# hpcaitech/CachedEmbedding

Hardware: AMD Instinct MI355X
Metric: embedding lookups/sec (cache op + EmbeddingBag fwd + bwd/SGD), Criteo-1TB table @1% cache (higher is better)
Workload: dtype f32

## Files before the change

cachedembedding_amd/_lib.py:

```python
from __future__ import annotations

import ctypes
import os
from ctypes import POINTER, Structure, c_char_p, c_double, c_float, c_int, c_int32, c_int64, c_size_t, c_uint64, c_void_p
from pathlib import Path

import torch

_PKG = Path(__file__).resolve().parent
LIB_PATH = Path(os.environ["CE_LIBRARY"]) if os.environ.get("CE_LIBRARY") else _PKG / "libce_hip.so"

CE_OK = 0
CE_ERR_INVALID = 1
CE_ERR_HIP = 2
CE_ERR_CAPACITY = 3
CE_ERR_NOMEM = 4
CE_ERR_UNSUPPORTED = 5
CE_ERR_RANGE = 6
CE_EVICT_DATASET = 0
CE_EVICT_LFU = 1
CE_EVICT_LRU = 2
CE_MODE_SUM = 0
CE_MODE_MEAN = 1
CE_ACT_F32 = 0
# ... 106 lines not shown
    "ce_bag_forward_src_keys_act": (c_int, _TABLE + [c_int64] + _KEYS + [c_void_p] + _ACT + _STREAM),
    "ce_bag_backward_dense_act": (c_int, _BAG + _ACT + _KEYS + _STREAM),
    "ce_bag_backward_sgd_act": (c_int, _BAG + _ACT + [c_float] + _KEYS + _STREAM),
    "ce_bag_backward_sgd_src_act": (c_int, _SRC + _ACT + [c_float] + _KEYS + [c_void_p] + _STREAM),
    "ce_bag_backward_dense_src_act": (c_int, _SRC + _ACT + _KEYS + _STREAM),
    "ce_bag_backward_rowwise_adagrad_act": (c_int, _BAG + _ACT + _ADAGRAD_TAIL),
    "ce_bag_backward_rowwise_adagrad_src_act": (c_int, _SRC + _ACT + _ADAGRAD_TAIL),
    "ce_host_fill_uniform_w16": (c_int, [c_void_p, c_int64, c_float, c_float, c_uint64, c_int32, c_int]),
    "ce_bag_forward_w16": (c_int, _W16 + _BAG[1:] + _ACT + _STREAM),
    "ce_bag_forward_src_keys_w16": (c_int, _W16 + [c_int64, c_int32, c_int64] + _KEYS + [c_void_p] + _ACT + _STREAM),
    "ce_bag_backward_w16_workspace": (c_size_t, [c_int64, c_int32]),
    "ce_bag_backward_update_w16": (c_int, _W16 + _BAG[1:] + _ACT + _W16_TAIL),
    "ce_bag_backward_update_src_w16": (c_int, _W16 + _SRC[1:] + _ACT + _W16_TAIL),
    "ce_bag_backward_update_sorted_workspace": (c_size_t, [c_int64, c_int64, c_int32]),
    "ce_bag_backward_update_sorted": (c_int, _W16 + _BAG[1:] + _ACT + _W16_TAIL[1:]),
    "ce_bag_backward_update_compact_workspace": (c_size_t, [c_int64, c_int64, c_int32]),
    "ce_bag_backward_update_compact": (c_int, _W16 + _BAG[1:] + _ACT + _W16_TAIL),
    "ce_bag_backward_update_compact_src": (c_int, _W16 + _SRC[1:] + _ACT + _W16_TAIL),
    "ce_bag_backward_sgd_lrdev": (c_int, _BAG + _ACT + [c_void_p] + _KEYS + _STREAM),
    "ce_bag_backward_sgd_src_lrdev": (c_int, _SRC + _ACT + [c_void_p] + _KEYS + [c_void_p] + _STREAM),
    "ce_bag_backward_update_lrdev": (c_int, _W16 + _BAG[1:] + _ACT + _LRDEV_TAIL),
    "ce_bag_backward_update_src_lrdev": (c_int, _W16 + _SRC[1:] + _ACT + _LRDEV_TAIL),
    "ce_q8_row_bytes": (c_size_t, [c_int32]),
    "ce_host_quantize_q8": (c_int, [c_void_p, c_int32, c_int64, c_int32, c_void_p, c_int]),
    "ce_host_dequantize_q8": (c_int, [c_void_p, c_int64, c_int32, c_void_p, c_int]),
    "ce_bag_forward_q8": (c_int, _BAG + _ACT + _STREAM),
    "ce_bag_forward_src_keys_q8": (c_int, _TABLE + [c_int64] + _KEYS + [c_void_p] + _ACT + _STREAM),
    "ce_q4_row_bytes": (c_size_t, [c_int32]),
    "ce_host_quantize_q4": (c_int, [c_void_p, c_int32, c_int64, c_int32, c_void_p, c_int]),
    "ce_host_dequantize_q4": (c_int, [c_void_p, c_int64, c_int32, c_void_p, c_int]),
    "ce_bag_forward_q4": (c_int, _BAG + _ACT + _STREAM),
    "ce_bag_forward_src_keys_q4": (c_int, _TABLE + [c_int64] + _KEYS + [c_void_p] + _ACT + _STREAM),
    "ce_cache_workspace_bytes": (c_size_t, [c_int64, c_int64, c_int64, c_int32]),
    "ce_cache_create": (c_int, [POINTER(CeCacheConfig), c_void_p, POINTER(c_void_p)]),
    "ce_cache_destroy": (c_int, [c_void_p]),
    "ce_cache_preload": (c_int, [c_void_p, c_void_p, c_void_p, c_int64, c_void_p]),
    "ce_cache_set_freq_bound": (c_int, [c_void_p, c_int64]),
    "ce_cache_prepare_ids": (c_int, [c_void_p, c_void_p, c_int64, c_void_p, c_void_p]),
    "ce_cache_prepare_ids_keys": (c_int, [c_void_p, c_void_p, c_int64, c_int64, c_void_p, c_int32, c_void_p, c_int32,
                                          c_int64, c_int64, c_int32, c_int64, c_void_p, c_void_p]),
    "ce_cache_prepare_ids_begin": (c_int, [c_void_p, c_void_p, c_int64, c_int64, c_void_p, c_int32, c_void_p, c_int32,
                                           c_int64, c_int64, c_int32, c_int64, c_void_p, c_void_p]),
    "ce_cache_prepare_ids_finish": (c_int, [c_void_p, c_void_p]),
    "ce_cache_prepare_ids_padded": (c_int, [c_void_p, c_void_p, c_int64, c_void_p, c_void_p]),
    "ce_cache_prepare_ids_begin_padded": (c_int, [c_void_p, c_void_p, c_int64, c_void_p, c_void_p]),
    "ce_cache_set_deferred_rows": (c_int, [c_void_p, c_int32]),
    "ce_cache_rows_ticket": (c_int64, [c_void_p]),
    "ce_cache_wait_rows": (c_int, [c_void_p, c_int64, c_void_p]),
    "ce_cache_last_stats": (c_int, [c_void_p, POINTER(CeCallStats)]),
    "ce_cache_totals": (c_int, [c_void_p, POINTER(c_int64), POINTER(c_int64), POINTER(c_int64),
                                POINTER(c_int64), POINTER(c_int64)]),
    "ce_cache_history": (c_int64, [c_void_p, c_int64, POINTER(CeCallStats), c_int64]),
    "ce_cache_lookup_slots": (c_int, [c_void_p, c_void_p, c_int64, c_void_p, c_void_p]),
    "ce_cache_flush": (c_int, [c_void_p, c_void_p]),
    "ce_cache_set_protect_depth": (c_int, [c_void_p, c_int32]),
    "ce_cache_set_transport": (c_int, [c_void_p, c_int32]),
    "ce_cache_get_transport": (c_int32, [c_void_p]),
    "ce_cache_set_cache_weight": (c_int, [c_void_p, c_void_p]),
    "ce_cache_graph_replayed": (c_int, [c_void_p, c_int64, c_int64, c_void_p]),
    "ce_cache_set_buffer_rows": (c_int, [c_void_p, c_int64]),
    "ce_cache_set_profiling": (c_int, [c_void_p, c_int32]),
    "ce_cache_phase_count": (c_int32, []),
    "ce_cache_phase_name": (c_char_p, [c_int32]),
    "ce_cache_phase_times": (c_int, [c_void_p, POINTER(c_double), c_int32, POINTER(c_int64), c_int32]),
    "ce_cache_writeback_wait": (c_int, [c_void_p]),
    "ce_cache_swap_stats": (c_int, [c_void_p, POINTER(c_double), POINTER(c_int64)]),
    "ce_cache_failures": (c_int, [c_void_p, POINTER(c_int64), POINTER(c_int32), POINTER(c_int64)]),
    "ce_cache_free_rows": (c_int, [c_void_p, POINTER(c_int64)]),
    "ce_bucketize_workspace": (c_size_t, [c_int64, c_int32]),
    "ce_bucketize_rows": (c_int, [c_void_p, c_int64, c_void_p, c_int32, c_void_p, c_void_p, c_void_p, c_void_p,
                                  c_size_t, c_void_p]),
    "ce_dedupe_bucket_rows": (c_int, [c_void_p, c_int64, c_void_p, c_int64, c_int32, c_void_p, c_void_p,
                                      c_void_p, c_void_p, c_void_p, c_void_p, c_void_p]),
    "ce_dedupe_bucket_rows_padded": (c_int, [c_void_p, c_int64, c_void_p, c_int64, c_int32, c_int64, c_void_p, c_void_p,
                                             c_void_p, c_void_p, c_void_p, c_void_p, c_void_p, c_void_p]),
    "ce_dedupe_bucket_rows_padded_window": (c_int, [c_void_p, c_int64, c_int64, c_void_p, c_int64, c_int32, c_int64,
                                                    c_void_p, c_void_p, c_void_p, c_void_p, c_void_p, c_void_p,
                                                    c_void_p, c_void_p]),
    "ce_exchange_local_index": (c_int, [c_void_p, c_int64, c_int64, c_void_p, c_int64, c_int64, c_int64, c_int64,
                                        c_void_p, c_void_p]),
    "ce_split_classify": (c_int, [c_void_p, c_int32, c_int32, c_int64, c_int64, c_void_p, c_int64, c_void_p, c_void_p,
                                  c_void_p]),
    "ce_split_places": (c_int, [c_void_p, c_void_p, c_int32, c_int32, c_int64, c_int32, c_void_p, c_void_p, c_void_p,
                                c_void_p, c_void_p, c_void_p]),
    "ce_exchange_local_index_split": (c_int, [c_void_p, c_int64, c_int64, c_void_p, c_void_p, c_void_p, c_int64, c_int64,
                                              c_int64, c_int64, c_int64, c_void_p, c_int32, c_int64, c_int64, c_int64,
                                              c_void_p, c_void_p, c_void_p]),
    "ce_bag_forward_max": (c_int, _LOOKUPS + [c_int64, c_void_p, c_void_p] + _STREAM),
    "ce_bag_backward_max": (c_int, [c_void_p, c_int64, c_int32, c_void_p, c_int64, c_int64, c_int64, c_void_p, c_void_p,
                                    c_float, c_void_p]),
    "ce_bag_backward_psw": (c_int, _LOOKUPS + [c_int64, c_void_p, c_void_p] + _STREAM),
    "ce_rows_renorm_workspace": (c_size_t, [c_int64]),
    "ce_rows_renorm": (c_int, [c_void_p, c_int64, c_int32, c_void_p, c_int64, c_float, c_float, c_void_p, c_size_t,
                               c_void_p]),
    "ce_rows_axpy": (c_int, [c_void_p, c_int64, c_int32, c_void_p, c_int64, c_void_p, c_float, c_void_p]),
}


class CeError(RuntimeError):
    def __init__(self, code: int, msg: str):
        super().__init__(f"libce_hip error {code}: {msg}")
        self.code = code


def _load() -> ctypes.CDLL:
    if not LIB_PATH.exists():
# ... 129 lines not shown
```

cachedembedding_amd/cache_mgr.py:

```python
from __future__ import annotations

import ctypes
import math
import weakref
from enum import Enum
from typing import List, Optional

import numpy as np
import torch

from . import _lib
from ._lib import CeCacheConfig, CeCallStats, check, lib, ptr, stream_ptr


class EvictionStrategy(Enum):
    LFU = 1
    DATASET = 2
    LRU = 3


EVICT_CODES = {EvictionStrategy.DATASET: _lib.CE_EVICT_DATASET, EvictionStrategy.LFU: _lib.CE_EVICT_LFU,
               EvictionStrategy.LRU: _lib.CE_EVICT_LRU}


# ... 100 lines not shown
            check(lib.ce_host_fill_uniform_w16(ctypes.c_void_p(self.host_ptr), self.tensor.numel(), lo, hi, seed,
                                               _lib.ACT_DTYPES[self.tensor.dtype], threads or _default_threads()))
            return self
        check(lib.ce_host_fill_uniform(ctypes.c_void_p(self.host_ptr), self.tensor.numel(), lo, hi, seed,
                                       threads or _default_threads()))
        return self


def _default_threads() -> int:
    import os
    return max(1, min(64, (os.cpu_count() or 1)))


class CachedParamMgr(torch.nn.Module):

    def __init__(self, weight, cuda_row_num: int = 0, buffer_size: int = 0, pin_weight: bool = True,
                 evict_strategy: EvictionStrategy = EvictionStrategy.DATASET, async_copy: bool = False,
                 device: Optional[torch.device] = None, strict: bool = True, use_idx_map: Optional[bool] = None):
        super().__init__()
        _lib.require_gpu()
        if cuda_row_num == 0:
            raise NotImplementedError("cuda_row_num == 0 (no cache) is not implemented")
        self._table = weight if isinstance(weight, HostTable) else HostTable.wrap(weight)
        self._weight = self._table.tensor
        self.num_embeddings, self._row_width = self._weight.shape
        self.quant_bits = self._table.quant_bits
        self.table_dtype = _lib.Q4 if self.quant_bits == 4 else self._weight.dtype
        q8 = self.quant_bits != 0
        self.embedding_dim = (2 * (self._row_width - _lib.CE_Q4_HEADER_BYTES) if self.quant_bits == 4
                              else self._row_width - _lib.CE_Q8_HEADER_BYTES) if q8 else self._row_width
        self._lib_dim = self._row_width // 4 if q8 else (
            self.embedding_dim // 2 if self.table_dtype in _lib.W16_DTYPES else self.embedding_dim)
        self.cuda_row_num = int(cuda_row_num)
        self.buffer_size = buffer_size
        self.pin_weight = pin_weight
        self._evict_strategy = evict_strategy
        self._async_copy = async_copy
        self.strict = strict
        self.device = torch.device(device) if device is not None else torch.device("cuda", torch.cuda.current_device())
        N, C, D = self.num_embeddings, self.cuda_row_num, self.embedding_dim
        assert N < 2 ** 31 - 1, "row ids are int32 on the device"
        dev = self.device
        self.cuda_cached_weight = torch.nn.Parameter(
            torch.zeros(C, self._row_width, device=dev, dtype=self._weight.dtype), requires_grad=not q8)
        self._idx_map: Optional[torch.Tensor] = None
        if use_idx_map:
            self._idx_map = torch.arange(N, device=dev, dtype=torch.int32)
        self.register_buffer("cached_idx_map", torch.empty(C, device=dev, dtype=torch.int32), persistent=False)
        self.register_buffer("inverted_cached_idx", torch.empty(N, device=dev, dtype=torch.int32), persistent=False)
        if evict_strategy == EvictionStrategy.LFU:
            self.register_buffer("freq_cnter", torch.empty(C, device=dev, dtype=torch.int64), persistent=False)
        else:
            self.freq_cnter = None
        self._max_ids = 2 ** 31 - 2
        self._deferred_rows = False
        self._handle = None
        self._workspace = None
        self._create_handle()
        self._hist_seen = 0
        self._failures_seen = 0
        self.num_hits_history: List[int] = []
        self.num_miss_history: List[int] = []
        self.num_write_back_history: List[int] = []

    def _create_handle(self):
        N, C = self.num_embeddings, self.cuda_row_num
        ws_bytes = lib.ce_cache_workspace_bytes(N, C, self._max_ids, self._lib_dim)
        self._workspace = torch.empty(ws_bytes + 256, dtype=torch.uint8, device=self.device)
        base = self._workspace.data_ptr()
        aligned = (base + 255) & ~255
        cfg = CeCacheConfig()
        cfg.num_embeddings = N
        cfg.cuda_row_num = C
        cfg.embedding_dim = self._lib_dim
        cfg.evict_strategy = EVICT_CODES[self._evict_strategy]
        tr = getattr(self, "_transport", None)
        cfg.transport = tr if tr is not None else (
            _lib.CE_TRANSPORT_STAGED if self._async_copy else _lib.CE_TRANSPORT_ZEROCOPY)
        reapply_worker = cfg.transport == _lib.CE_TRANSPORT_WORKER
        if reapply_worker:
            cfg.transport = _lib.CE_TRANSPORT_ZEROCOPY
        cfg.protect_depth = 0
        cfg.max_ids_per_call = self._max_ids
        cfg.host_weight = self._table.host_ptr
        cfg.host_weight_dev = self._table.dev_ptr
        cfg.cache_weight = self.cuda_cached_weight.data_ptr()
        cfg.idx_map = ptr(self._idx_map)
        cfg.inverted_cached_idx = self.inverted_cached_idx.data_ptr()
        cfg.cached_idx_map = self.cached_idx_map.data_ptr()
        cfg.freq_cnter = ptr(self.freq_cnter)
        cfg.workspace = aligned
        cfg.workspace_bytes = ws_bytes
        h = ctypes.c_void_p()
        with torch.cuda.device(self.device):
            check(lib.ce_cache_create(ctypes.byref(cfg), stream_ptr(), ctypes.byref(h)))
        self._handle = h
        self._fin = weakref.finalize(self, lib.ce_cache_destroy, h)
        if self.buffer_size and self.buffer_size > 0:
            check(lib.ce_cache_set_buffer_rows(h, int(self.buffer_size)))
        if reapply_worker:
            self.set_transport("worker")

    @property
    def weight(self) -> torch.Tensor:
        if self._handle is not None:
            check(lib.ce_cache_writeback_wait(self._handle))
        return self._weight

    @property
    def idx_map(self) -> torch.Tensor:
        if self._idx_map is None:
            return torch.arange(self.num_embeddings, device=self.device, dtype=torch.int32)
        return self._idx_map

    @property
    def cuda_available_row_num(self) -> int:
        out = ctypes.c_int64()
        check(lib.ce_cache_free_rows(self._handle, ctypes.byref(out)))
        return out.value

    @torch.no_grad()
    def reorder(self, ids_freq_mapping=None, warmup_ratio: float = 0.7):
        N, C = self.num_embeddings, self.cuda_row_num
        freq = None
        order = None
        if ids_freq_mapping is not None:
            freq = torch.as_tensor(ids_freq_mapping).to(device=self.device, dtype=torch.int64).view(-1)
            assert freq.numel() == N
            order = torch.argsort(freq, descending=True, stable=True)
            if self._evict_strategy == EvictionStrategy.DATASET:
                inv = torch.empty(N, device=self.device, dtype=torch.int32)
                inv[order] = torch.arange(N, device=self.device, dtype=torch.int32)
                if self._idx_map is None:
                    self._idx_map = inv
                    self._recreate_with_idx_map()
                else:
                    self._idx_map.copy_(inv)
        n = min(int(math.ceil(C * warmup_ratio)), N)
        if n > 0:
            rows = None
            fvals = None
            if self._evict_strategy in (EvictionStrategy.LFU, EvictionStrategy.LRU) and freq is not None:
                rows = order[:n].to(torch.int32).contiguous()
                if self._evict_strategy == EvictionStrategy.LFU:
                    fvals = freq[order[:n]].contiguous()
            with torch.cuda.device(self.device):
                check(lib.ce_cache_preload(self._handle, ptr(rows), ptr(fvals), n, stream_ptr()))
                if fvals is not None:
                    check(lib.ce_cache_set_freq_bound(self._handle, int(fvals.max().item())))
                torch.cuda.current_stream().synchronize()

    def _recreate_with_idx_map(self):
        assert self.cuda_available_row_num == self.cuda_row_num, "reorder() after rows were cached"
        self._fin.detach()
        lib.ce_cache_destroy(self._handle)
        self._create_handle()
        self._hist_seen = 0
        self._failures_seen = 0

    @torch.no_grad()
    def prepare_ids(self, ids: torch.Tensor, out: Optional[torch.Tensor] = None, padded: bool = False,
                    defer_rows: bool = False) -> torch.Tensor:
        assert ids.is_cuda, "ids must live on the GPU (recsys/dlrm_main.py:250 moves the batch first)"
        shape = ids.shape
        flat = ids if (ids.dim() == 1 and ids.dtype == torch.int64 and ids.is_contiguous()) \
            else ids.reshape(-1).long().contiguous()
        if out is None:
            slots = torch.empty_like(flat)
        else:
            assert out.is_cuda and out.dtype == torch.int64 and out.is_contiguous() and out.numel() == flat.numel()
            slots = out if out.dim() == 1 else out.view(-1)
        fn = lib.ce_cache_prepare_ids_padded if padded else lib.ce_cache_prepare_ids
        if torch.cuda.current_device() == self.device.index:
            check(fn(self._handle, ptr(flat), flat.numel(), ptr(slots), stream_ptr()))
        else:
            with torch.cuda.device(self.device):
                check(fn(self._handle, ptr(flat), flat.numel(), ptr(slots), stream_ptr()))
        if self._deferred_rows and not defer_rows:
            self.wait_rows()
        self._strict_check()
        return slots if slots.shape == shape else slots.view(shape)

    def _strict_check(self) -> None:
        if self.strict and not torch.cuda.is_current_stream_capturing():
            st = CeCallStats()
            rc = lib.ce_cache_last_stats(self._handle, ctypes.byref(st))
            self._pull_history()
            if rc != _lib.CE_OK:
                self._failures_seen += 1
            if rc == _lib.CE_ERR_CAPACITY:
                raise AssertionError(_lib.last_error())
            if rc == _lib.CE_ERR_RANGE:
                raise IndexError(_lib.last_error())
            check(rc)

    @torch.no_grad()
    def prepare_ids_begin(self, ids: torch.Tensor, out: torch.Tensor, keys_out: Optional[torch.Tensor] = None, **layout):
        return self.prepare_ids_keys(ids, out, keys_out, _begin_only=True, **layout)

    @torch.no_grad()
    def prepare_ids_begin_padded(self, ids: torch.Tensor, out: torch.Tensor) -> torch.Tensor:
        assert ids.is_cuda and ids.dtype == torch.int64 and ids.is_contiguous()
        assert out.is_cuda and out.dtype == torch.int64 and out.is_contiguous() and out.numel() == ids.numel()
# ... 232 lines not shown
```

cachedembedding_amd/cached_embedding.py:

```python
from __future__ import annotations

from typing import Callable, Iterator, List, Optional, Tuple, Union

import torch
import torch.nn as nn

from . import _lib
from .cache_mgr import CachedParamMgr, EvictionStrategy, HostTable
from .functional import FusedRowwiseAdagrad, FusedSGD, check_accumulator, check_lr, check_lr_path, embedding_bag


def _refuse_q8_update(module, what: str, lr) -> None:
    if lr is not None and getattr(module, "table_dtype", None) == _lib.Q8:
        raise NotImplementedError(f"{what}(lr) with a q8 (torch.uint8) table: a quantized table is never updated")
    if lr is not None and getattr(module, "table_dtype", None) == _lib.Q4:
        raise NotImplementedError(f"{what}(lr) with a q4 (torch.quint4x2) table: a quantized table is never updated")


def _quant_name(bits: int) -> str:
    return "q4 (torch.quint4x2)" if bits == 4 else "q8 (torch.uint8)"


class CachedEmbeddingBag(nn.Module):
    def __init__(self, num_embeddings: int, embedding_dim: int, padding_idx: Optional[int] = None,
# ... 41 lines not shown
            if padding_idx > 0:
                assert padding_idx < num_embeddings, "Padding_idx must be within num_embeddings"
            elif padding_idx < 0:
                assert padding_idx >= -num_embeddings, "Padding_idx must be within num_embeddings"
                padding_idx = num_embeddings + padding_idx
        self.padding_idx = padding_idx
        self.max_norm = max_norm
        self.norm_type = norm_type
        self.scale_grad_by_freq = scale_grad_by_freq
        self.sparse = sparse
        self.mode = mode
        self.include_last_offset = include_last_offset
        self.evict_strategy = evict_strategy
        self.cache_ratio = cache_ratio
        self.cuda_row_num = int(num_embeddings * cache_ratio) if cuda_row_num is None else int(cuda_row_num)
        self.pool_str = mode
        self.cache_op = True
        self.fused_sgd = FusedSGD(None)
        self.fused_adagrad = FusedRowwiseAdagrad(None)

        if _table is not None:
            table = _table
            assert table.tensor.dtype == (torch.uint8 if q8 else self.table_dtype) and table.quant_bits == bits \
                and table.tensor.shape[0] == num_embeddings
        elif q8:
            w = _weight.detach()
            if w.dtype == torch.uint8:
                width = _lib.q4_row_bytes(embedding_dim) if bits == 4 else _lib.q8_row_bytes(embedding_dim)
                assert tuple(w.shape) == (num_embeddings, width)
                table = HostTable.wrap(w if w.device.type == "cpu" and w.is_contiguous() else w.cpu().contiguous(),
                                       quant_bits=bits)
            else:
                assert tuple(w.shape) == (num_embeddings, embedding_dim)
                if w.dtype not in _lib.ACT_DTYPES:
                    w = w.float()
                table = HostTable.allocate(num_embeddings, embedding_dim, dtype=self.table_dtype).quantize_from(
                    w.cpu().contiguous())
        elif _weight is None:
            table = HostTable.allocate(num_embeddings, embedding_dim, dtype=self.table_dtype)
            table.fill_uniform_(-1.0 / num_embeddings, 1.0 / num_embeddings, init_seed)
            if padding_idx is not None:
                table.tensor[padding_idx].zero_()
        else:
            w = _weight.detach()
            assert tuple(w.shape) == (num_embeddings, embedding_dim)
            if w.device.type != "cpu" or w.dtype != self.table_dtype or not w.is_contiguous():
                w = w.to("cpu", self.table_dtype).contiguous()
            table = HostTable.wrap(w)
        self.cache_weight_mgr = CachedParamMgr(table, self.cuda_row_num, buffer_size, pin_weight,
                                               evict_strategy=evict_strategy, device=device, strict=strict,
                                               use_idx_map=True if _idx_map is not None else None)
        if _idx_map is not None:
            self.cache_weight_mgr._idx_map.copy_(_idx_map)
        self.cache_weight_mgr.reorder(ids_freq_mapping, warmup_ratio)
        if q8:
            self.eval()
        if w16:
            self.set_weight_rounding(self.weight_rounding, self.weight_rounding_seed)

    @property
    def weight(self) -> torch.Tensor:
        return self.cache_weight_mgr.weight

    def named_parameters(self, prefix: str = "", recurse: bool = True, remove_duplicate: bool = True
                         ) -> Iterator[Tuple[str, nn.Parameter]]:
        yield (prefix + ("." if prefix else "") + "weight", self.cache_weight_mgr.cuda_cached_weight)

    def parameters(self, recurse: bool = True) -> Iterator[nn.Parameter]:
        yield self.cache_weight_mgr.cuda_cached_weight

    def set_cache_op(self, cache_op: bool = True):
        self.cache_op = cache_op

    def set_cache_mgr_async_copy(self, flag: bool):
        self.cache_weight_mgr.set_async_copy(flag)

    def set_fused_sgd(self, lr: Union[float, torch.Tensor, None], deterministic: bool = False,
                      accumulator: str = "cache"):
        _refuse_q8_update(self, "set_fused_sgd", lr)
        if isinstance(lr, torch.Tensor):
            check_lr_path(check_lr(lr), bool(deterministic), self.mode)
        if lr is not None or accumulator != "step":
            check_accumulator("sgd", self.table_dtype, accumulator, bool(deterministic), self.weight_rounding)
        if lr is not None and self.fused_adagrad.lr is not None:
            raise ValueError("fused row-wise Adagrad is set: set_fused_rowwise_adagrad(None) before set_fused_sgd(lr)")
        if lr is not None and deterministic and self.table_dtype != torch.float32:
            raise NotImplementedError("FusedSGD(deterministic=True) with a 16-bit table")
        self.fused_sgd.lr = lr
        self.fused_sgd.deterministic = deterministic
        self.fused_sgd.accumulator = accumulator

    def set_fused_rowwise_adagrad(self, lr: Union[float, torch.Tensor, None], eps: float = 1e-8,
                                  deterministic: bool = False, accumulator: str = "cache"):
        _refuse_q8_update(self, "set_fused_rowwise_adagrad", lr)
        if isinstance(lr, torch.Tensor):
            check_lr_path(check_lr(lr), bool(deterministic), self.mode)
        if lr is not None or accumulator != "step":
            check_accumulator("rowwise_adagrad", self.table_dtype, accumulator, bool(deterministic),
                              self.weight_rounding)
        if lr is not None and self.fused_sgd.lr is not None:
            raise ValueError("fused SGD is set: set_fused_sgd(None) before set_fused_rowwise_adagrad(lr)")
        mgr = self.cache_weight_mgr
        if lr is not None and getattr(mgr, "momentum1", None) is None:
            mgr.momentum1 = torch.zeros(mgr.num_embeddings, device=mgr.device, dtype=torch.float32)
        self.fused_adagrad.lr = lr
        self.fused_adagrad.eps = float(eps)
# ... 112 lines not shown
```

cachedembedding_amd/csrc/ce_bag.hip:

```cpp
#include <algorithm>

#include "ce_common.h"

namespace ce {

struct BagParams {
  const float* weight;
  float* dst;
  const void* grad_out;
  const int64_t* indices;
  const void* offsets;
  const float* psw;
  int64_t nnz;
  int32_t num_bags;
  int32_t rowlen;
  int32_t g_log2;
  int32_t off64;
  int32_t include_last;
  int32_t mode;
  int32_t hookF;
  int32_t hookB;
  float alpha;
  int32_t pad0;
  uint32_t num_rows;
// ... 373 lines not shown
__device__ __forceinline__ void tile_sort_1024(KT (&key)[4], KT* lds, int tid) {
  for (int k = 2; k <= kBwdTile; k <<= 1) {
    for (int j = k >> 1; j > 0; j >>= 1) {
      if (j >= 256) {
#pragma unroll
        for (int r = 0; r < 4; ++r) lds[tid * 4 + r] = key[r];
        __syncthreads();
#pragma unroll
        for (int r = 0; r < 4; ++r) {
          const int i = tid * 4 + r;
          const KT other = lds[i ^ j];
          const bool lower = (i & j) == 0, up = (i & k) == 0;
          const KT lo = key[r] < other ? key[r] : other, hi = key[r] < other ? other : key[r];
          key[r] = (lower == up) ? lo : hi;
        }
        __syncthreads();
      } else if (j >= 4) {
#pragma unroll
        for (int r = 0; r < 4; ++r) {
          const int i = tid * 4 + r;
          const KT other = shfl_xor_key<KT>(key[r], j >> 2);
          const bool lower = (i & j) == 0, up = (i & k) == 0;
          const KT lo = key[r] < other ? key[r] : other, hi = key[r] < other ? other : key[r];
          key[r] = (lower == up) ? lo : hi;
        }
      } else {
#pragma unroll
        for (int r = 0; r < 4; ++r) {
          if (r & j) continue;
          const bool up = ((tid * 4 + r) & k) == 0;
          const KT a = key[r], b = key[r | j];
          if ((a > b) == up) {
            key[r] = b;
            key[r | j] = a;
          }
        }
      }
    }
  }
#pragma unroll
  for (int r = 0; r < 4; ++r) lds[tid * 4 + r] = key[r];
  __syncthreads();
}

constexpr int kSegLen = 16384;
constexpr int kSegKeys = 16;
#ifndef CE_SEG_BUCKETS
#define CE_SEG_BUCKETS 8192
#endif
constexpr int kSegBuckets = CE_SEG_BUCKETS;
constexpr int kExclRun = 32;
constexpr unsigned kExclFlag = 0x80000000u;

template <bool SRC, bool EXCL, bool ROWS>
__global__ __launch_bounds__(1024) void k_bag_presort_seg(const int64_t* __restrict__ indices, int64_t nnz_per_batch,
                                                         int32_t segs_per_batch, int64_t n_segs, uint32_t num_rows,
                                                         unsigned long long* __restrict__ keys_out, BagParams lay,
                                                         int64_t off_stride, const int64_t* __restrict__ ids,
                                                         int64_t* __restrict__ ids_minmax, int64_t* slots_io,
                                                         const int32_t* __restrict__ inverted,
                                                         const int* __restrict__ status) {
  __shared__ unsigned long long lk[kSegLen];
  static_assert(sizeof(unsigned long long) * kSegLen <= 160 * 1024 - 1024, "gfx950: 160 KB of LDS per CU");
  int* const cnt = (int*)lk;
  __shared__ int wsum[16];
  __shared__ long long mm_s[2][16];
  const int tid = threadIdx.x, lane = tid & 63, wv = tid >> 6;
  for (int64_t seg = blockIdx.x; seg < n_segs; seg += gridDim.x) {
    const int64_t batch = seg / segs_per_batch;
    const int sib = (int)(seg - batch * segs_per_batch);
    const int64_t in_base = batch * nnz_per_batch + (int64_t)sib * kSegLen;
    const int64_t base = seg * kSegLen;
    const int n_here = (int)min((int64_t)kSegLen, nnz_per_batch - (int64_t)sib * kSegLen);
    BagParams q = lay;
    if (SRC && lay.offsets) q.offsets = (const char*)lay.offsets + batch * off_stride * (lay.off64 ? 8 : 4);
    for (int i = tid; i <= kSegBuckets; i += 1024) cnt[i] = 0;
    __syncthreads();
    unsigned long long key[kSegKeys];
    int place[kSegKeys], bkt[kSegKeys];
    int32_t slot_r[ROWS ? kSegKeys : 1];
    if (ROWS) {
      const bool failed = *status != CE_OK;
      int32_t row_r[kSegKeys];
#pragma unroll
      for (int r = 0; r < kSegKeys; ++r) {
        const int e = r * 1024 + tid;
        row_r[r] = e < n_here ? (int32_t)slots_io[in_base + e] : -1;
      }
#pragma unroll
      for (int r = 0; r < kSegKeys; ++r) slot_r[r] = (row_r[r] >= 0 && !failed) ? inverted[row_r[r]] : -1;
#pragma unroll
      for (int r = 0; r < kSegKeys; ++r) {
        const int e = r * 1024 + tid;
        if (e < n_here) slots_io[in_base + e] = (int64_t)slot_r[r];
      }
    }
#pragma unroll
    for (int r = 0; r < kSegKeys; ++r) {
      const int e = r * 1024 + tid;
      key[r] = ~0ull;
      bkt[r] = kSegBuckets;
      if (e < n_here) {
        const int64_t row = ROWS ? (int64_t)slot_r[ROWS ? r : 0] : indices[in_base + e];
        const bool valid = (uint64_t)row < (uint64_t)num_rows;
        if (valid || SRC) {
          unsigned low = (unsigned)e;
          if (SRC)
            low = (unsigned)out_row(q, lay.offsets ? find_bag(q, sib * kSegLen + e) : sib * kSegLen + e);
          key[r] = ((unsigned long long)(valid ? (uint32_t)row : 0xffffffffu) << 32) | low;
          if (valid) bkt[r] = (int)(row & (kSegBuckets - 1));
        }
      }
      const int b0 = __builtin_amdgcn_readfirstlane(bkt[r]);
      if (__all(bkt[r] == b0)) {
        int first = 0;
        if (lane == 0) first = atomicAdd(&cnt[b0], 64);
        place[r] = __shfl(first, 0) + lane;
      } else {
        place[r] = atomicAdd(&cnt[bkt[r]], 1);
      }
    }
    __syncthreads();
    constexpr int kPer = kSegBuckets / 1024;
    int c4[kPer], sum = 0;
#pragma unroll
    for (int q = 0; q < kPer; ++q) { c4[q] = cnt[tid * kPer + q]; sum += c4[q]; }
    int inc = sum;
#pragma unroll
    for (int d = 1; d < 64; d <<= 1) {
      const int o = __shfl_up(inc, d);
      if (lane >= d) inc += o;
    }
    if (lane == 63) wsum[wv] = inc;
    __syncthreads();
    int pre = inc - sum;
    for (int k = 0; k < wv; ++k) pre += wsum[k];
    int total = 0;
    for (int k = 0; k < 16; ++k) total += wsum[k];
#pragma unroll
    for (int q = 0; q < kPer; ++q) { cnt[tid * kPer + q] = pre; pre += c4[q]; }
    if (tid == 0) cnt[kSegBuckets] = total;
    __syncthreads();
    if (!EXCL) {
// ... 937 lines not shown
  return launch_fwd_keys(weight, kTableQ8, num_rows, dim, true, nnz, src_keys, out, act_dtype, (hipStream_t)stream);
}

#define CE_REQUIRE_Q4_DIM(dim)                                                         \
  CE_REQUIRE(ce_q4_row_bytes(dim) != 0, CE_ERR_UNSUPPORTED,                            \
             "a q4 table needs dim %% 32 == 0 and 32 <= dim <= 1024 (got %d)", (int)(dim))
#define CE_REQUIRE_Q4_ALIGNED(weight, out, act)                                        \
  CE_REQUIRE(al16(weight) && act_aligned(out, act), CE_ERR_INVALID,                    \
             "a q4 table must be 16-byte aligned and its output on the vector boundary")

extern "C" int ce_bag_forward_q4(const void* weight, int64_t num_rows, int32_t dim, const int64_t* indices, int64_t nnz,
                                 const void* offsets, int32_t offsets_are_i64, int64_t num_bags,
                                 int32_t include_last_offset, const float* per_sample_weights, int32_t mode,
                                 int64_t hook_features, void* out, int32_t act_dtype, ce_stream_t stream) {
  CE_REQUIRE_ACT(act_dtype);
  CE_REQUIRE_Q4_DIM(dim);
  if (num_bags == 0) return CE_OK;
  CE_REQUIRE(weight && out && (indices || nnz == 0), CE_ERR_INVALID, "null pointer");
  CE_REQUIRE(offsets || num_bags == nnz, CE_ERR_INVALID,
             "offsets == NULL states one id per bag (offsets = arange): num_bags must equal nnz");
  CE_REQUIRE_Q4_ALIGNED(weight, out, act_dtype);
  BagParams p{};
  RowGeom r;
  int rc = fill_params(p, r, dim, true, indices, nnz, offsets, offsets_are_i64, num_bags, include_last_offset,
                       per_sample_weights, mode, hook_features);
  if (rc) return rc;
  return launch_fwd(p, r, weight, kTableQ4, num_rows, out, act_dtype, (hipStream_t)stream);
}

extern "C" int ce_bag_forward_src_keys_q4(const void* weight, int64_t num_rows, int32_t dim, int64_t nnz,
                                          const uint64_t* src_keys, void* out, int32_t act_dtype, ce_stream_t stream) {
  CE_REQUIRE_ACT(act_dtype);
  CE_REQUIRE_Q4_DIM(dim);
  if (nnz == 0) return CE_OK;
  CE_REQUIRE(weight && src_keys && out, CE_ERR_INVALID, "null pointer");
  CE_REQUIRE_ROWS(num_rows);
  CE_REQUIRE_Q4_ALIGNED(weight, out, act_dtype);
  return launch_fwd_keys(weight, kTableQ4, num_rows, dim, true, nnz, src_keys, out, act_dtype, (hipStream_t)stream);
}

extern "C" int64_t ce_bag_presort_len(int64_t nnz) { return nnz <= 0 ? 0 : padded_keys(nnz); }

static int window_layout(BagParams& lay, const BagLayout& L, const int64_t* indices, int64_t nnz_per_batch) {
  CE_REQUIRE(L.num_bags > 0 && L.offsets_batch_stride >= 0, CE_ERR_INVALID, "bad offsets");
  CE_REQUIRE(L.offsets || L.num_bags == nnz_per_batch, CE_ERR_INVALID,
             "offsets may only be NULL for the one-id-per-bag layout (num_bags == nnz_per_batch)");
  RowGeom unused;
  return fill_params(lay, unused, 4, true, indices, nnz_per_batch, L.offsets, L.offsets_are_i64, L.num_bags,
                     L.include_last_offset, nullptr, CE_MODE_SUM, L.hook_features);
}

static int launch_presort(const int64_t* indices, int64_t* slots_io, const int32_t* inverted, const int* status,
                          int64_t nnz_per_batch, int64_t n_batches, int64_t num_rows, const BagLayout* L,
                          const int64_t* ids, int64_t* ids_minmax, uint64_t* keys_out, hipStream_t s) {
  if (nnz_per_batch == 0 || n_batches == 0) return CE_OK;
  CE_REQUIRE((slots_io ? inverted && status : indices != nullptr) && keys_out && nnz_per_batch > 0 && n_batches > 0,
             CE_ERR_INVALID, "bad arguments");
  CE_REQUIRE(nnz_per_batch < (int64_t)INT32_MAX - kSegLen, CE_ERR_INVALID, "batch too large");
  CE_REQUIRE_ROWS(num_rows);
  const int64_t spb = cdiv(nnz_per_batch, kSegLen);
  const int64_t nseg = spb * n_batches;
  CE_REQUIRE(spb < (int64_t)INT32_MAX && nseg < (int64_t)INT32_MAX, CE_ERR_INVALID, "too many segments");
  BagParams lay{};
  if (L) {
    int rc = window_layout(lay, *L, indices, nnz_per_batch);
    if (rc) return rc;
  }
  const dim3 grid((unsigned)std::min<int64_t>(nseg, kMaxBlocks)), block(1024);
  const int64_t off_stride = L ? L->offsets_batch_stride : 0;
  auto launch = [&](auto src, auto excl, auto rows) {
    hipLaunchKernelGGL((k_bag_presort_seg<decltype(src)::value, decltype(excl)::value, decltype(rows)::value>), grid, block,
                       0, s, indices, nnz_per_batch, (int32_t)spb, nseg, (uint32_t)num_rows,
                       (unsigned long long*)keys_out, lay, off_stride, ids, ids_minmax, slots_io, inverted, status);
  };
  const std::true_type yes{};
  const std::false_type no{};
  if (slots_io && L) launch(yes, no, yes);
  else if (slots_io) launch(no, no, yes);
  else if (L && ids_minmax) launch(yes, yes, no);
  else if (L) launch(yes, no, no);
  else launch(no, no, no);
  CE_LAUNCH_CHECK();
  return CE_OK;
}

namespace ce {
int presort_window_from_rows(int64_t* slots_io, int64_t nnz_per_batch, int64_t n_batches, int64_t num_rows,
                             const int32_t* inverted, const int* status, int32_t src_keys, const BagLayout& lay,
                             uint64_t* keys_out, hipStream_t stream) {
  return launch_presort(nullptr, slots_io, inverted, status, nnz_per_batch, n_batches, num_rows, src_keys ? &lay : nullptr,
                        nullptr, nullptr, keys_out, stream);
}
}

extern "C" int ce_bag_presort_window(const int64_t* indices, int64_t nnz_per_batch, int64_t n_batches,
                                     int64_t num_rows, uint64_t* keys_out, ce_stream_t stream) {
  return launch_presort(indices, nullptr, nullptr, nullptr, nnz_per_batch, n_batches, num_rows, nullptr, nullptr, nullptr,
                        keys_out, (hipStream_t)stream);
}

static int presort_window_src_impl(const int64_t* indices, int64_t nnz_per_batch, int64_t n_batches, int64_t num_rows,
                                   const BagLayout& L, const int64_t* ids, uint64_t* keys_out, int64_t* seg_id_ranges,
                                   ce_stream_t stream) {
  if (nnz_per_batch == 0 || n_batches == 0) return CE_OK;
  BagParams lay{};
  int rc = window_layout(lay, L, indices, nnz_per_batch);
  if (rc) return rc;
  return launch_presort(indices, nullptr, nullptr, nullptr, nnz_per_batch, n_batches, num_rows, &L, ids, seg_id_ranges,
                        keys_out, (hipStream_t)stream);
}

extern "C" int ce_bag_presort_window_src(const int64_t* indices, int64_t nnz_per_batch, int64_t n_batches,
                                         int64_t num_rows, const void* offsets, int32_t offsets_are_i64,
                                         int64_t offsets_batch_stride, int64_t num_bags, int32_t include_last_offset,
                                         int64_t hook_features, uint64_t* keys_out, ce_stream_t stream) {
  return presort_window_src_impl(indices, nnz_per_batch, n_batches, num_rows,
                                 {offsets, offsets_are_i64, offsets_batch_stride, num_bags, include_last_offset, hook_features},
                                 nullptr, keys_out, nullptr, stream);
}

extern "C" int ce_bag_presort_window_src_excl(const int64_t* indices, int64_t nnz_per_batch, int64_t n_batches,
                                              int64_t num_rows, const void* offsets, int32_t offsets_are_i64,
                                              int64_t offsets_batch_stride, int64_t num_bags,
                                              int32_t include_last_offset, int64_t hook_features, const int64_t* ids,
                                              uint64_t* keys_out, int64_t* seg_id_ranges, ce_stream_t stream) {
  CE_REQUIRE(seg_id_ranges, CE_ERR_INVALID, "null seg_id_ranges");
  return presort_window_src_impl(indices, nnz_per_batch, n_batches, num_rows,
                                 {offsets, offsets_are_i64, offsets_batch_stride, num_bags, include_last_offset, hook_features},
                                 ids, keys_out, seg_id_ranges, stream);
}

extern "C" int ce_bag_presort(const int64_t* indices, int64_t nnz, int64_t num_rows, uint64_t* keys_out,
                              ce_stream_t stream) {
  return ce_bag_presort_window(indices, nnz, 1, num_rows, keys_out, stream);
}

extern "C" int ce_rows_axpy(float* weight, int64_t num_rows, int32_t dim, const int64_t* index, int64_t n,
                            const float* src_rows, float alpha, ce_stream_t stream) {
  if (n == 0) return CE_OK;
  CE_REQUIRE(weight && index && src_rows, CE_ERR_INVALID, "null pointer");
  CE_REQUIRE(dim > 0 && n > 0 && n < (int64_t)INT32_MAX, CE_ERR_INVALID, "bad sizes");
  CE_REQUIRE_ROWS(num_rows);
  RowGeom r;
  int rc = row_geometry(dim, al16(weight) && al16(src_rows), r);
// ... 36 lines not shown
```

cachedembedding_amd/csrc/ce_cache.hip:

```cpp
#include <sched.h>
#include <stdlib.h>
#include <string.h>
#include <sys/prctl.h>

#include <algorithm>
#include <atomic>
#include <chrono>
#include <condition_variable>
#include <functional>
#include <mutex>
#include <thread>
#include <vector>

#include "ce_common.h"

#include "ce_cache_index.h"
#include "ce_cache_select.h"
#include "ce_cache_rows.h"
#include "ce_cache_fused.h"
#include "ce_cache_worker.h"


struct KeysTail {
  int64_t n_batches, nnz_per_batch;
// ... 10 lines not shown
  ce::Ctl* ctl = nullptr;
  uint32_t* bitmap = nullptr;
  int32_t *blk_unique = nullptr, *blk_miss = nullptr, *coarse = nullptr, *miss_list = nullptr, *slot_epoch = nullptr,
          *victims = nullptr, *blk_free = nullptr, *free_list = nullptr;
  int32_t* miss_list_b[2] = {};
  int32_t* free_list_b[2] = {};
  ce::ChainWords* chain = nullptr;
  unsigned long long *lb_emit = nullptr, *lb_remap = nullptr;
  unsigned lb_tag = 0;
  ce::FrontWords* front = nullptr;
  int32_t *fine_cnt = nullptr, *coarse_cnt = nullptr;
  long long front_calls = 0;
  bool front_cleanup_pending = false;
  unsigned long long* keys = nullptr;
  uint32_t* hist = nullptr;
  ce_call_stats_t* ring = nullptr;
  ce_call_stats_t* ring_dev = nullptr;
  hipEvent_t ev = nullptr;
  float* stage = nullptr;
  int32_t* stage_idx = nullptr;
  long long seq = 0;
  long long drained = 0;
  std::vector<ce_call_stats_t> history;
  int64_t cpu_to_cuda_numel = 0, cuda_to_cpu_numel = 0, cache_miss = 0, total_cache = 0;
  int vec = 0;
  int rowlen = 0, g_log2 = 0, slot_bits = 0, word_bits = 0;
  int host_threads = 1;
  float* stage_dev = nullptr;
  float* stage_host = nullptr;
  int32_t* list_host = nullptr;
  ce::Ctl* ctl_host = nullptr;
  int64_t stage_rows = 0;
  int64_t list_rows = 0;
  int64_t buffer_rows = 0;
  ce::RowPool* pool = nullptr;
  ce::SwapEngine* wb = nullptr;
  unsigned long long* evt_keys[2] = {};
  int32_t* evt_pos[2] = {};
  uint32_t evt_mask = 0;
  float* stage2 = nullptr;
  int32_t* stage_idx2 = nullptr;
  float* in_stage = nullptr;
  long long hist_base = 1;
  ce::PhaseProf* prof = nullptr;
  uint64_t freq_bound = 0;
  uint64_t graph_freq_limit = ~0ull;
  bool freq_bound_known = true;
  long long n_failed = 0;
  int last_fail_status = CE_OK;
  long long last_fail_seq = 0;
  bool free_zero = false;
  long long free_reset_seq = 0;
  bool deferred_rows = false;
  struct Pending {
    bool active = false;
    int64_t n = 0;
    int64_t* slots_out = nullptr;
    hipStream_t s = nullptr;
    bool worker = false, capturing = false, has_tail = false;
    bool chained = false;
    long long call = 0;
    int parity = 0;
    long long in_job = 0, seq_arg = 0;
    int cap_groups = 1, swap_threads = 256;
    bool sel_pending = false;
    bool sel_steady = false;
    long long sel_out_job = 0;
    int sel_wbuf = 0;
    int pslot = 0, pmark = 0;
    const void* prof = nullptr;
    KeysTail tail{};
  } pend;
};

using namespace ce;

template <typename VT_> struct RowTag { typedef VT_ VT; };
template <typename F> static inline void for_rows(const ce_cache* h, F&& f) {
  if (h->vec) f(RowTag<f32x4>{}); else f(RowTag<float>{});
}

static PhaseProf* live_prof(const ce_cache* h) {
  return (h->prof && (const void*)h->prof == h->pend.prof) ? h->prof : nullptr;
}
static void phase_mark(ce_cache* h) {
  ce_cache::Pending& x = h->pend;
  if (PhaseProf* const prof = live_prof(h)) (void)hipEventRecord(prof->ev[x.pslot][x.pmark++], x.s);
}

static int ensure_writeback(ce_cache* h);

static void drain(ce_cache* h) {
  while (h->drained < h->seq) {
    const long long s = h->drained + 1;
    const ce_call_stats_t& r = h->ring[s % kRing];
    if (r.seq != s) break;
    if (h->history.empty()) h->hist_base = s;
    h->history.push_back(r);
    if (h->history.size() > (size_t)2 * kHistoryKeep) {
      h->history.erase(h->history.begin(), h->history.end() - kHistoryKeep);
      h->hist_base = h->history.front().seq;
    }
    if (r.status != CE_OK) {
      h->n_failed += 1;
      h->last_fail_status = r.status;
      h->last_fail_seq = s;
      h->free_zero = false;
      h->free_reset_seq = h->seq;
    } else if (r.kind == CE_CALL_PREPARE && s > h->free_reset_seq) {
      h->free_zero = r.n_free_after == 0;
    }
    if (r.status == CE_OK && r.kind != CE_CALL_PRELOAD) {
      h->cpu_to_cuda_numel += r.n_miss * h->cfg.embedding_dim;
      h->cuda_to_cpu_numel += r.n_evict * h->cfg.embedding_dim;
      h->cache_miss += r.miss_lookups;
      h->total_cache += r.n_ids;
      if (h->wb && h->wb->chained && r.kind == CE_CALL_PREPARE) {
        std::lock_guard<std::mutex> g(h->wb->m);
        h->wb->in_rows += r.n_miss;
      }
    }
    h->drained = s;
  }
}

static hipEvent_t last_rows_event(ce_cache* h) {
  if (!h->wb || !h->wb->chained || h->wb->chain_calls == 0) return nullptr;
  return h->wb->ev_rows[h->wb->chain_calls % SwapEngine::kRowsRing];
}
static int join_rows(ce_cache* h, hipStream_t s) {
  if (hipEvent_t ev = last_rows_event(h)) CE_HIP_CHECK(hipStreamWaitEvent(s, ev, 0));
  return CE_OK;
}
// ... 314 lines not shown
    static const int out_threads = [] { const char* e = getenv("CE_WB_THREADS"); return e ? atoi(e) : dflt; }();
    static const int in_threads = [] { const char* e = getenv("CE_GATHER_THREADS"); return e ? atoi(e) : dflt; }();
    w->out_pool = new RowPool(std::max(1, std::min(out_threads, 64)));
    w->in_pool = new RowPool(std::max(1, std::min(in_threads, 64)));
    w->rowlen = h->rowlen;
    w->g_log2 = h->g_log2;
    w->vec = h->vec;
    w->out_thread = std::thread([w] { w->run_out(); });
    if (!w->chained) w->in_thread = std::thread([w] { w->run_in(); });
  } while (0);
  if (rc) {
    delete w;
    set_error("swap worker setup failed (pinned buffers / streams / events)");
    return rc;
  }
  h->wb = w;
  return CE_OK;
}

extern "C" int ce_cache_set_freq_bound(ce_cache_t* h, int64_t bound) {
  CE_REQUIRE(h && bound >= 0, CE_ERR_INVALID, "bad bound");
  if (h->cfg.evict_strategy == CE_EVICT_LRU) return CE_OK;
  h->freq_bound = std::max<uint64_t>(h->freq_bound, (uint64_t)bound);
  h->freq_bound_known = true;
  return CE_OK;
}

extern "C" int ce_cache_preload(ce_cache_t* h, const int32_t* rows, const int64_t* freq_vals, int64_t n,
                                ce_stream_t stream) {
  CE_REQUIRE(h, CE_ERR_INVALID, "null handle");
  CE_REQUIRE(n >= 0 && n <= h->cfg.cuda_row_num, CE_ERR_INVALID, "preload count out of range");
  CE_REQUIRE(!h->pend.active, CE_ERR_INVALID, "a cache op begun with ce_cache_prepare_ids_begin has not been finished");
  if (n == 0) return CE_OK;
  if (freq_vals && h->cfg.evict_strategy != CE_EVICT_LRU) h->freq_bound_known = false;
  int rc = before_call(h);
  if (rc) return rc;
  if (h->wb) {
    rc = h->wb->wait_out(h->wb->out_issued);
    if (rc) return rc;
  }
  hipStream_t s = (hipStream_t)stream;
  const ce_cache_config_t& c = h->cfg;
  rc = join_rows(h, s);
  if (rc) return rc;
  h->seq += 1;
  const int64_t groups_per_block = 256 >> h->g_log2;
  for_rows(h, [&](auto r) {
    using VT = typename decltype(r)::VT;
    hipLaunchKernelGGL((k_admit<VT>), dim3(grid_for(n, (int)groups_per_block * kSwapRows)), dim3(256), 0, s, rows,
                       (const int32_t*)nullptr, (const long long*)nullptr, (long long)n, (const VT*)c.host_weight_dev,
                       (VT*)c.cache_weight, h->rowlen, h->g_log2, (const Ctl*)nullptr, 0ll);
  });
  hipLaunchKernelGGL(k_admit_maps, dim3(grid_for(n, 256)), dim3(256), 0, s, rows, (const int32_t*)nullptr,
                     (const long long*)nullptr, (long long)n, c.cached_idx_map, c.inverted_cached_idx,
                     c.freq_cnter, freq_vals, h->slot_epoch, kEpochNever, (Ctl*)nullptr,
                     (ce_call_stats_t*)nullptr, 0ll, (const unsigned long long*)nullptr, 0ll);
  hipLaunchKernelGGL(k_preload_end, dim3(1), dim3(1), 0, s, (long long)n, h->ctl, h->ring_dev + (h->seq % kRing),
                     h->seq);
  CE_LAUNCH_CHECK();
  CE_HIP_CHECK(hipEventRecord(h->ev, s));
  return CE_OK;
}

static int worker_selftest(ce_cache* h, hipStream_t s) {
  SwapEngine* w = h->wb;
  if (w->tested && w->tested_stream == s) return CE_OK;
  CE_HIP_CHECK(hipStreamSynchronize(s));
  unsigned long long* word = w->sig + 2;
  __atomic_store_n(word, 0ull, __ATOMIC_RELEASE);
  CE_HIP_CHECK(hipStreamWaitValue64(s, word, 1, hipStreamWaitValueGte, ~0ull));
  std::this_thread::sleep_for(std::chrono::milliseconds(2));
  hipError_t e = hipMemcpyAsync(w->rows_host[0], w->stage_dev[0], 64, hipMemcpyDeviceToHost, w->out_stream);
  if (e == hipSuccess) e = hipMemcpyAsync(w->rows_host[1], w->stage_dev[1], 64, hipMemcpyDeviceToHost, w->out_stream2);
  if (e == hipSuccess) e = hipMemcpyAsync(w->in_stage_dev, w->rows_host[0], 64, hipMemcpyHostToDevice, w->in_stream);
  bool done = e == hipSuccess;
  if (done) {
    for (hipStream_t st : {w->out_stream, w->out_stream2, w->in_stream})
      if (stream_wait_polite(st, 0.25) != hipSuccess) done = false;
  }
  __atomic_store_n(word, 1ull, __ATOMIC_RELEASE);
  CE_HIP_CHECK(hipStreamSynchronize(s));
  if (e != hipSuccess) {
    set_error("worker transport self-test: %s", hipGetErrorString(e));
    return CE_ERR_HIP;
  }
  if (!done) {
    set_error("worker transport self-test failed: copies on the library's copy streams do not run while the cache-op "
              "stream is parked in hipStreamWaitValue64 (they share a hardware queue with it: GPU_MAX_HW_QUEUES = %s)",
              getenv("GPU_MAX_HW_QUEUES") ? getenv("GPU_MAX_HW_QUEUES") : "unset");
    return CE_ERR_UNSUPPORTED;
  }
  w->tested = true;
  w->tested_stream = s;
  return CE_OK;
}

struct FrontTail {
  const int32_t* miss_tmp;
  const FrontWords* fw;
  uint32_t* bitmap;
  int32_t *fine, *coarse;
};
static FrontTail take_front_tail(ce_cache* h) {
  if (!h->front_cleanup_pending) return FrontTail{nullptr, nullptr, nullptr, nullptr, nullptr};
  h->front_cleanup_pending = false;
  return FrontTail{h->victims, h->front + (h->front_calls & 1), h->bitmap, h->fine_cnt, h->coarse_cnt};
}
// ... 15 lines not shown
    if (capturing) {
      bound = h->freq_bound + kGraphFreqHeadroom;
      h->graph_freq_limit = bound;
    } else {
      h->freq_bound = bound;
    }
    const int bits = 64 - __builtin_clzll(bound | 1ull) + h->slot_bits;
    top_pass = h->freq_bound_known ? std::min(kLevels - 1, std::max(0, (bits + kDigitBits - 1) / kDigitBits - 1))
                                   : kLevels - 1;
  }
  return top_pass;
}

static int launch_keys_hist(ce_cache* h) {
  const ce_cache::Pending& x = h->pend;
  const ce_cache_config_t& c = h->cfg;
  const int64_t N = c.num_embeddings, C = c.cuda_row_num;
  const int top_pass = select_top_pass(h, x.n, x.capturing);
  const FrontTail ft = take_front_tail(h);
  const auto keys_kernel = c.evict_strategy == CE_EVICT_LRU   ? k_keys<CE_EVICT_LRU>
                           : c.evict_strategy == CE_EVICT_LFU ? k_keys<CE_EVICT_LFU>
                                                              : k_keys<CE_EVICT_DATASET>;
  hipLaunchKernelGGL(keys_kernel, dim3(std::min(grid_for(C, 256 * 4), 512)), dim3(256), 0, x.s, c.cached_idx_map, c.freq_cnter,
                     h->slot_epoch, C, N, x.seq_arg, c.protect_depth, h->slot_bits, top_pass, h->keys, h->hist, h->ctl,
                     ft.miss_tmp, ft.fw, ft.bitmap, ft.fine, ft.coarse, (int)h->L.n_chunks);
  const int hgrid = (int)std::min<int64_t>(kNumCU, std::max<int64_t>(1, cdiv(C, 1024 * 4)));
  for (int pass = top_pass - 1; pass >= 0; --pass)
    hipLaunchKernelGGL(k_hist, dim3(hgrid), dim3(1024), 0, x.s, h->keys, C, pass, top_pass, h->hist, h->ctl);
  return top_pass;
}


static int64_t staged_chunk(const ce_cache* h, int64_t rows) {
  return (h->buffer_rows > 0 && h->buffer_rows < rows) ? h->buffer_rows : rows;
}
static size_t rowbytes(const ce_cache* h) { return (size_t)h->cfg.embedding_dim * sizeof(float); }

static int staged_swap(ce_cache* h, hipStream_t s) {
  const ce_cache_config_t& c = h->cfg;
  const int D = c.embedding_dim;
  if (!h->ctl_host) CE_HIP_CHECK(hipHostMalloc((void**)&h->ctl_host, sizeof(Ctl), hipHostMallocDefault));
  CE_HIP_CHECK(hipMemcpyAsync(h->ctl_host, h->ctl, sizeof(Ctl), hipMemcpyDeviceToHost, s));
  CE_HIP_CHECK(hipStreamSynchronize(s));
  const Ctl ctl = *h->ctl_host;
  if (ctl.status != CE_OK) return CE_OK;
  const int64_t k = ctl.k_evict, m = ctl.n_miss;
  const int64_t big = std::max<int64_t>(std::max(k, m), 1);
  int rc = ensure_staging(h, staged_chunk(h, big), big);
  if (rc) return rc;
  const int gpb = 256 >> h->g_log2;
  if (k > 0) {
    int32_t* evicted_rows_dev = h->free_list;
    hipLaunchKernelGGL(k_evict_maps, dim3(grid_for(k, 256)), dim3(256), 0, s, h->victims, c.cached_idx_map,
                       c.inverted_cached_idx, evicted_rows_dev, h->ctl);
    CE_HIP_CHECK(hipMemcpyAsync(h->list_host, evicted_rows_dev, (size_t)k * 4, hipMemcpyDeviceToHost, s));
    const int64_t chunk = staged_chunk(h, k);
    for (int64_t off = 0; off < k; off += chunk) {
      const int64_t cnt = std::min(chunk, k - off);
      for_rows(h, [&](auto r) {
        using VT = typename decltype(r)::VT;
        hipLaunchKernelGGL((k_pack_rows<VT>), dim3(grid_for(cnt, gpb)), dim3(256), 0, s, (const int32_t*)h->victims + off,
                           (long long)cnt, (const VT*)c.cache_weight, (VT*)h->stage_dev, h->rowlen, h->g_log2);
      });
      CE_HIP_CHECK(hipMemcpyAsync(h->stage_host, h->stage_dev, (size_t)cnt * rowbytes(h), hipMemcpyDeviceToHost, s));
      CE_HIP_CHECK(hipStreamSynchronize(s));
      float* table = c.host_weight;
      const float* st = h->stage_host;
      const int32_t* rows = h->list_host + off;
      const size_t rb = rowbytes(h);
      host_pool(h)->parallel(cnt, [=](int64_t lo, int64_t hi) {
        for (int64_t i = lo; i < hi; ++i) memcpy(table + (size_t)rows[i] * D, st + (size_t)i * D, rb);
      });
    }
  }
  return CE_OK;
}

static int admit_staged(ce_cache* h) {
  const ce_cache_config_t& c = h->cfg;
  hipStream_t s = h->pend.s;
  const Ctl ctl = *h->ctl_host;
  const int64_t m = (ctl.status == CE_OK) ? ctl.n_miss : 0;
  if (m <= 0) return CE_OK;
  const int D = c.embedding_dim, gpb = 256 >> h->g_log2;
  const size_t rb = rowbytes(h);
  CE_HIP_CHECK(hipMemcpyAsync(h->list_host, h->miss_list, (size_t)m * 4, hipMemcpyDeviceToHost, s));
  CE_HIP_CHECK(hipStreamSynchronize(s));
  const float* table = c.host_weight;
  float* st = h->stage_host;
  const int64_t chunk = staged_chunk(h, m);
  for (int64_t off = 0; off < m; off += chunk) {
    const int64_t cnt = std::min(chunk, m - off);
    if (off > 0) CE_HIP_CHECK(hipStreamSynchronize(s));
    const int32_t* rows = h->list_host + off;
    host_pool(h)->parallel(cnt, [=](int64_t lo, int64_t hi) {
      for (int64_t i = lo; i < hi; ++i) memcpy(st + (size_t)i * D, table + (size_t)rows[i] * D, rb);
    });
    CE_HIP_CHECK(hipMemcpyAsync(h->stage_dev, h->stage_host, (size_t)cnt * rb, hipMemcpyHostToDevice, s));
    for_rows(h, [&](auto r) {
      using VT = typename decltype(r)::VT;
      hipLaunchKernelGGL((k_unpack_rows<VT>), dim3(grid_for(cnt, gpb)), dim3(256), 0, s, (const int32_t*)h->free_list + off,
                         (long long)cnt, (const VT*)h->stage_dev, (VT*)c.cache_weight, h->rowlen, h->g_log2);
    });
  }
  return CE_OK;
}

static int select_and_stage(ce_cache* h) {
  const ce_cache::Pending& x = h->pend;
  const ce_cache_config_t& c = h->cfg;
  const Layout& L = h->L;
  const int64_t C = c.cuda_row_num;
  hipStream_t s = x.s;
  const bool worker = x.worker, steady = x.sel_steady;
  const int wbuf = x.sel_wbuf, n_vblocks = (int)cdiv(C, 4096), gpb = 256 >> h->g_log2;
  int32_t* const free_list = h->free_list_b[x.chained ? x.parity : 0];
  const int top_pass = launch_keys_hist(h);
  hipLaunchKernelGGL(k_victims, dim3((unsigned)n_vblocks), dim3(256), 0, s, h->keys, C, h->victims, L.list_cap, h->ctl,
                     (const uint32_t*)h->hist, top_pass, h->ring_dev, x.seq_arg, steady ? h->blk_free : (int32_t*)nullptr);
  phase_mark(h);
  if (c.transport == CE_TRANSPORT_ZEROCOPY || worker) {
    float* const stage_cur = (worker && wbuf) ? h->stage2 : h->stage;
    int32_t* const stage_idx_cur = (worker && wbuf) ? h->stage_idx2 : h->stage_idx;
    const long long scap = (long long)L.stage_rows;
    const int sgrid = (int)std::min<int64_t>(512, std::max<int64_t>(1, cdiv(L.stage_rows, gpb)));
    WbMail* const mail = worker ? h->wb->mail_dev + wbuf : nullptr;
    const dim3 sg(sgrid + (steady ? n_vblocks : 0));
    const EvTable evt = (worker && h->wb->chained) ? EvTable{h->evt_keys[wbuf], h->evt_pos[wbuf], h->evt_mask}
                                                     : EvTable{nullptr, nullptr, 0u};
    for_rows(h, [&](auto r) {
      using VT = typename decltype(r)::VT;
      hipLaunchKernelGGL((k_evict_stage<VT>), sg, dim3(256), 0, s, h->victims, c.cached_idx_map, c.inverted_cached_idx,
                         (const VT*)c.cache_weight, (VT*)stage_cur, stage_idx_cur, scap, h->rowlen, h->g_log2, h->ctl, mail,
                         x.sel_out_job, sgrid, (const unsigned long long*)h->keys, C, (const int32_t*)h->blk_free, free_list,
                         evt, L.list_cap > L.stage_rows ? (VT*)c.host_weight_dev : (VT*)nullptr);
    });
    if (worker) {
      CE_HIP_CHECK(hipEventRecord(h->wb->out_ev[wbuf], s));
      h->wb->push_out();
    }
  } else {
    const int rc = staged_swap(h, s);
    if (rc) return rc;
  }
  phase_mark(h);
  if (steady) {
  } else if (C <= 16384) {
    hipLaunchKernelGGL(k_free_single, dim3(1), dim3(1024), 0, s, c.cached_idx_map, C, free_list, h->ctl);
  } else {
    hipLaunchKernelGGL(k_free_count, dim3((unsigned)L.n_slot_blocks), dim3(256), 0, s, c.cached_idx_map, C,
                       h->blk_free, h->ctl);
    hipLaunchKernelGGL(k_free_emit, dim3((unsigned)L.n_slot_blocks), dim3(256), 0, s, c.cached_idx_map, C,
                       h->blk_free, free_list, h->ctl);
  }
  phase_mark(h);
  return CE_OK;
}

struct MarkCfg {
  bool merge;
  int u, threads, blocks, hot_words;
};
static MarkCfg mark_cfg(const ce_cache* h, int64_t n) {
  const bool ranked = h->cfg.idx_map != nullptr;
  MarkCfg m;
  m.merge = !ranked;
  m.threads = ranked ? 512 : 256;
  m.hot_words = (int)std::min<int64_t>(h->L.bitmap_words, ranked ? 8192 : 2048);
  m.u = n >= 65536 ? 4 : 1;
  m.blocks = std::min(grid_for(n, m.threads * m.u), 256);
  return m;
}

constexpr int64_t kScanMaxIds = (1 << 23) - 1;

static void launch_front_kernels(ce_cache* h, const int64_t* ids, int64_t n, int64_t* slots_out, hipStream_t s,
                                 int allow_pad, bool steady, long long seq_arg, int32_t* miss_list, WbMail* mail_in,
                                 long long in_job, int32_t* miss_host, long long* n_admit_out, bool single_pass_ok) {
  const ce_cache_config_t& c = h->cfg;
  const Layout& L = h->L;
  const int64_t N = c.num_embeddings, C = c.cuda_row_num;
  if (h->front_cleanup_pending) {
    hipLaunchKernelGGL(k_front_cleanup, dim3(64), dim3(256), 0, s, (const int32_t*)h->victims,
                       (const FrontWords*)(h->front + (h->front_calls & 1)), h->bitmap, h->fine_cnt, h->coarse_cnt,
                       (int)L.n_chunks);
    h->front_cleanup_pending = false;
  }
  if (single_pass_ok && !mail_in && !miss_host && n < (int64_t)INT32_MAX && L.n_chunks <= kRankMaxChunks) {
    const long long fc = ++h->front_calls;
    FrontWords* const fw = h->front + (fc & 1);
    FrontWords* const fw_next = h->front + ((fc + 1) & 1);
    if (n > 0) {
      const int U = n >= 65536 ? 2 : 1;
      const int threads = (int)std::min<int64_t>(1024, std::max<int64_t>(64, cdiv(cdiv(n, U), 64) * 64));
      const dim3 tg((unsigned)cdiv(n, (int64_t)threads * U)), tb(threads);
#define CE_TOUCH(U_)                                                                                                \
  hipLaunchKernelGGL((k_touch<U_>), tg, tb, 0, s, ids, n, c.idx_map, c.inverted_cached_idx, N, h->bitmap, h->fine_cnt, \
                     h->coarse_cnt, h->slot_epoch, seq_arg, fw, h->victims, (unsigned)L.list_cap, slots_out, allow_pad)
      if (U == 2) CE_TOUCH(2); else CE_TOUCH(1);
#undef CE_TOUCH
    }
    const int rgrid = (int)std::min<int64_t>(kNumCU, std::max<int64_t>(1, cdiv(std::max(n, C), 4096)));
    hipLaunchKernelGGL(k_miss_rank, dim3(rgrid), dim3(256), (size_t)L.n_chunks * 4, s, (const int32_t*)h->victims, fw, fw_next,
                       (const uint32_t*)h->bitmap, (const int32_t*)h->fine_cnt, (const int32_t*)h->coarse_cnt,
                       (int)L.n_chunks, (unsigned)L.list_cap, miss_list, (const int32_t*)h->slot_epoch, C, h->hist, seq_arg, h->ctl, n, h->ring_dev,
                       (long long)L.stage_rows, steady ? 1 : 0, n_admit_out);
    h->front_cleanup_pending = true;
    return;
  }
  hipLaunchKernelGGL(k_begin, dim3(16), dim3(256), 0, s, h->ctl, h->coarse,
                     (int)(((L.n_chunks >> kCoarseShift) + 1) * 2 * kCoarsePad), h->hist, seq_arg);
  if (n > 0) {
    const MarkCfg mc = mark_cfg(h, n);
    const dim3 mg(mc.blocks), mb(mc.threads);
#define CE_MARK(M, U_)                                                                                             \
  hipLaunchKernelGGL((k_mark<M, U_>), mg, mb, mc.hot_words * 4, s, ids, n, c.idx_map, c.inverted_cached_idx, N,    \
                     h->word_bits, mc.hot_words, h->bitmap, h->ctl, slots_out, allow_pad)
    if (mc.merge) { if (mc.u == 4) CE_MARK(true, 4); else CE_MARK(true, 1); }
    else { if (mc.u == 4) CE_MARK(false, 4); else CE_MARK(false, 1); }
#undef CE_MARK
  }
  hipLaunchKernelGGL(k_count, dim3((unsigned)L.n_chunks), dim3(256), 0, s, (const uint4*)h->bitmap,
                     c.inverted_cached_idx, N, h->blk_unique, h->blk_miss, h->coarse);
  hipLaunchKernelGGL(k_emit, dim3((unsigned)cdiv(L.n_chunks, kEmitSub)), dim3(256), 0, s, (uint4*)h->bitmap, c.inverted_cached_idx, N,
                     h->blk_miss, h->coarse, (int)L.n_chunks, miss_list, h->slot_epoch, seq_arg, h->ctl, C, n, h->ring_dev,
                     mail_in, in_job, (long long)L.stage_rows, miss_host, steady ? 1 : 0, n_admit_out);
}

static int prepare_ids_second_half(ce_cache* h);
static int chained_second_half(ce_cache* h);
static int launch_slots_keys(ce_cache* h);

static ce_cache::Pending& record_call(ce_cache* h, int64_t n, int64_t* slots_out, hipStream_t s, const KeysTail* tail,
                                      bool worker, bool capturing, int split, long long out_job, long long in_job,
                                      long long chain_call) {
  const ce_cache_config_t& c = h->cfg;
  ce_cache::Pending x;
  x.n = n;
  x.slots_out = slots_out;
  x.s = s;
  x.worker = worker;
  x.capturing = capturing;
  x.has_tail = tail != nullptr;
  if (tail) x.tail = *tail;
  x.chained = chain_call > 0;
  x.call = chain_call;
  x.parity = (int)(chain_call & 1);
  x.in_job = in_job;
  x.seq_arg = capturing ? 0ll : (long long)h->seq;
  const int swap_blocks = c.protect_depth > 0 ? 32 : 512;
  x.swap_threads = 256;
  x.cap_groups = (int)std::min<int64_t>(swap_blocks, std::max<int64_t>(1, cdiv(h->L.list_cap, (x.swap_threads >> h->g_log2) * kSwapRows)));
// ... 28 lines not shown
  {
    const int blocks = n <= 600000 ? 32 : 20;
    const long long prev = out_job - 1;
    const int pb = (int)(prev & 1);
    bool landed;
    {
      std::lock_guard<std::mutex> g(w->m);
      landed = w->out_done >= prev;
      w->in_jobs += 1;
      if (!landed) w->in_probed += 1;
    }
    const bool has_prev = prev >= w->probe_floor && !landed;
    const unsigned long long* ek = has_prev ? h->evt_keys[pb] : nullptr;
    const long long* n_ptr = &h->chain->n_admit[parity];
    for_rows(h, [&](auto r) {
      using VT = typename decltype(r)::VT;
      hipLaunchKernelGGL((k_admit_probe<VT>), dim3(blocks), dim3(1024), 0, w->in_stream, h->miss_list_b[parity], n_ptr,
                         (const VT*)h->cfg.host_weight_dev, (VT*)h->in_stage, h->rowlen, h->g_log2, ek,
                         (const int32_t*)h->evt_pos[pb], h->evt_mask, (uint32_t)prev, (const VT*)(pb ? h->stage2 : h->stage));
    });
  }
  phase_mark(h);
  if (split) {
    x.active = true;
    CE_LAUNCH_CHECK();
    return CE_OK;
  }
  return chained_second_half(h);
}

static int chained_second_half(ce_cache* h) {
  ce_cache::Pending& x = h->pend;
  x.active = false;
  x.sel_pending = false;
  SwapEngine* const w = h->wb;
  const ce_cache_config_t& c = h->cfg;
  const Layout& L = h->L;
  hipStream_t s = x.s;
  const int parity = x.parity, wbuf = x.sel_wbuf, pslot = x.pslot;
  const long long call = x.call, out_job = x.sel_out_job;
  PhaseProf* const prof = live_prof(h);
  if (prof) {
    (void)hipEventRecord(prof->resume[pslot], s);
    prof->resumed[pslot] = true;
  }
  if (call > 1) CE_HIP_CHECK(hipStreamWaitEvent(s, w->ev_rows[(call - 1) % SwapEngine::kRowsRing], 0));
  hipEvent_t sel_done = w->out_ev[wbuf];
  if (x.sel_steady && x.n <= kScanMaxIds) {
    const int64_t C = c.cuda_row_num;
    const int top_pass = launch_keys_hist(h);
    phase_mark(h);
    StageArgs a;
    a.cached_idx_map = c.cached_idx_map;
    a.inverted = c.inverted_cached_idx;
    a.freq = c.freq_cnter;
    a.slot_epoch = h->slot_epoch;
    a.C = C;
    a.seq_arg = x.seq_arg;
    a.top_pass = top_pass;
    a.keys = h->keys;
    a.hist = h->hist;
    a.ctl = h->ctl;
    a.lb = h->lb_remap;
    h->lb_tag = (h->lb_tag + 1) & 0xffffu;
    a.tag = h->lb_tag;
    a.free_list = h->free_list_b[parity];
    a.miss_list = h->miss_list_b[parity];
    a.ring = h->ring_dev;
    a.n_unpack_out = &h->chain->n_unpack[parity];
    a.cache = c.cache_weight;
    a.stage = wbuf ? h->stage2 : h->stage;
    a.stage_rows_idx = wbuf ? h->stage_idx2 : h->stage_idx;
    a.scap = (long long)L.stage_rows;
    a.rowlen = h->rowlen;
    a.g_log2 = h->g_log2;
    a.vec = h->vec;
    a.mail = w->mail_dev + wbuf;
    a.job = out_job;
    a.evt = EvTable{h->evt_keys[wbuf], h->evt_pos[wbuf], h->evt_mask};
    a.host_overflow = L.list_cap > L.stage_rows ? (void*)c.host_weight_dev : nullptr;
    hipLaunchKernelGGL(k_rank_victims, dim3((unsigned)cdiv(C, kRemapSlots)), dim3(256), 0, s, a);
    {
      const int gpb = 256 >> h->g_log2;
      const int sgrid = (int)std::min<int64_t>(x.n <= 600000 ? 256 : 512,
                                               std::max<int64_t>(1, cdiv(L.stage_rows, gpb * kStageRowsInFlight)));
      hipLaunchKernelGGL(k_stage_maps, dim3(sgrid), dim3(256), 0, s, a);
    }
    CE_HIP_CHECK(hipEventRecord(w->out_ev[wbuf], s));
    w->push_out();
    for (int j = 0; j < 2; ++j) phase_mark(h);
  } else {
    int rc0 = select_and_stage(h);
    if (rc0) return rc0;
    hipLaunchKernelGGL(k_admit_maps, dim3(grid_for(L.list_cap, 256)), dim3(256), 0, s, h->miss_list_b[parity],
                       h->free_list_b[parity], (const long long*)&h->ctl->n_miss, 0ll, c.cached_idx_map,
                       c.inverted_cached_idx, c.freq_cnter, (const int64_t*)nullptr, h->slot_epoch, 0, h->ctl,
                       h->ring_dev, x.seq_arg, (const unsigned long long*)nullptr, 0ll, &h->chain->n_unpack[parity]);
    CE_HIP_CHECK(hipEventRecord(w->ev_miss[parity], s));
    sel_done = w->ev_miss[parity];
  }
  CE_HIP_CHECK(hipStreamWaitEvent(w->in_stream, sel_done, 0));
  {
    const int gpb = 256 >> h->g_log2;
    const int ugrid = (int)std::min<int64_t>(x.n <= 600000 ? 128 : 512, std::max<int64_t>(1, cdiv(L.stage_rows, gpb)));
    const long long prev = out_job - 1;
    const int pb = (int)(prev & 1);
    const unsigned long long* ek = prev >= w->probe_floor ? h->evt_keys[pb] : nullptr;
    const bool tail_possible = L.list_cap > L.stage_rows;
    for_rows(h, [&](auto r) {
      using VT = typename decltype(r)::VT;
      hipLaunchKernelGGL((k_unpack_chained<VT>), dim3(ugrid), dim3(256), 0, w->in_stream, h->free_list_b[parity],
                         (const long long*)&h->chain->n_unpack[parity], (long long)L.stage_rows, (const VT*)h->in_stage,
                         (VT*)c.cache_weight, h->rowlen, h->g_log2, (const int32_t*)h->miss_list_b[parity],
                         tail_possible ? (const VT*)c.host_weight_dev : (const VT*)nullptr, ek,
                         (const int32_t*)h->evt_pos[pb], h->evt_mask, (uint32_t)prev, (const VT*)(pb ? h->stage2 : h->stage));
    });
  }
  if (prof) (void)hipEventRecord(prof->adm1[pslot], w->in_stream);
  hipEvent_t rows = w->ev_rows[call % SwapEngine::kRowsRing];
  CE_HIP_CHECK(hipEventRecord(rows, w->in_stream));
  phase_mark(h);
  int rc = launch_slots_keys(h);
  if (rc) return rc;
  if (prof) prof->pending[pslot] = true;
  CE_LAUNCH_CHECK();
  if (!h->deferred_rows) CE_HIP_CHECK(hipStreamWaitEvent(s, rows, 0));
  CE_HIP_CHECK(hipEventRecord(h->ev, s));
  return CE_OK;
}

static int prepare_ids_impl(ce_cache_t* h, const int64_t* ids, int64_t n, int64_t* slots_out, ce_stream_t stream,
                            int allow_pad, const KeysTail* tail = nullptr, int split = 0) {
  CE_REQUIRE(h, CE_ERR_INVALID, "null handle");
  CE_REQUIRE(!h->pend.active, CE_ERR_INVALID, "a cache op begun with ce_cache_prepare_ids_begin has not been finished");
  CE_REQUIRE(n >= 0 && n <= std::max<int64_t>(h->cfg.max_ids_per_call, 0), CE_ERR_INVALID,
             "n=%lld exceeds max_ids_per_call=%lld", (long long)n, (long long)h->cfg.max_ids_per_call);
  CE_REQUIRE(n == 0 || (ids && slots_out), CE_ERR_INVALID, "null ids/slots");
  hipStream_t s = (hipStream_t)stream;
  hipStreamCaptureStatus cap_st = hipStreamCaptureStatusNone;
  if (s != nullptr) CE_HIP_CHECK(hipStreamIsCapturing(s, &cap_st));
  const bool capturing = cap_st == hipStreamCaptureStatusActive;
  if (capturing) {
    CE_REQUIRE(h->cfg.transport == CE_TRANSPORT_ZEROCOPY, CE_ERR_UNSUPPORTED,
               "only the zero-copy transport can be captured in a hipGraph (the others hand rows to host threads)");
    CE_REQUIRE(!h->prof, CE_ERR_UNSUPPORTED, "switch the phase timers off before capturing a cache op");
    CE_REQUIRE(!split, CE_ERR_UNSUPPORTED, "a cache op in two halves cannot be captured in a hipGraph");
  }
  int rc = capturing ? CE_OK : before_call(h);
  if (rc) return rc;
  bool worker = h->cfg.transport == CE_TRANSPORT_WORKER;
  if (worker) {
    rc = ensure_writeback(h);
    if (rc) return rc;
    if (h->wb->chained) {
      rc = h->wb->check();
      if (rc) return rc;
      h->seq += 1;
      return chained_first_half(h, ids, n, slots_out, s, allow_pad, tail, split);
    }
  }
  if (!capturing) h->seq += 1;

  long long out_job = 0, in_job = 0;
  if (worker) {
    rc = worker_selftest(h, s);
    if (rc == CE_ERR_UNSUPPORTED) {
      fprintf(stderr, "[libce_hip] %s -- falling back to the zero-copy transport\n", ce_last_error());
      rc = h->wb->wait_out(h->wb->out_issued);
      if (rc) return rc;
      h->cfg.transport = CE_TRANSPORT_ZEROCOPY;
      worker = false;
    } else if (rc) {
      return rc;
    }
  }
  if (worker) {
    {
      int prio = 0, prio_lo = 0, prio_hi = 0;
      (void)hipDeviceGetStreamPriorityRange(&prio_lo, &prio_hi);
      if (s != nullptr && prio_hi != prio_lo && hipStreamGetPriority(s, &prio) == hipSuccess)
        CE_REQUIRE(prio != prio_hi, CE_ERR_UNSUPPORTED,
                   "the worker transport's host-gather admission cannot run its cache op on a highest-priority stream "
                   "(its copy streams use that priority to stay out of the parked stream's hardware queue)");
    }
    out_job = h->wb->out_issued + 1;
    in_job = h->wb->in_issued + 1;
    rc = h->wb->wait_out(out_job - 2);
    if (rc == CE_OK) rc = h->wb->wait_in(in_job - 2);
    if (rc) return rc;
  }
  ce_cache::Pending& x = record_call(h, n, slots_out, s, tail, worker, capturing, split, out_job, in_job, 0ll);
  if (PhaseProf* const prof = live_prof(h)) prof->collect(x.pslot);
  phase_mark(h);
  launch_front_kernels(h, ids, n, slots_out, s, allow_pad, x.sel_steady, x.seq_arg, h->miss_list,
                       worker ? h->wb->mail_dev + 2 : (WbMail*)nullptr, in_job,
                       worker ? h->wb->miss_host_dev : (int32_t*)nullptr, (long long*)nullptr, !capturing);
  if (worker) {
    CE_HIP_CHECK(hipEventRecord(h->wb->in_ev[in_job & 1], s));
    h->wb->push_in(out_job - 1);
  }
  phase_mark(h);
  if (!x.sel_pending) {
    rc = select_and_stage(h);
    if (rc) return rc;
  }
  if (split) {
    x.active = true;
    CE_LAUNCH_CHECK();
    return CE_OK;
  }
  return prepare_ids_second_half(h);
}

static int launch_slots_keys(ce_cache* h) {
  const ce_cache::Pending& x = h->pend;
  const ce_cache_config_t& c = h->cfg;
  const int64_t C = c.cuda_row_num, n = x.n;
  int64_t* const slots_out = x.slots_out;
  hipStream_t s = x.s;
  const ce_stream_t stream = (ce_stream_t)s;
  const int lfu = c.evict_strategy == CE_EVICT_LFU;
  const KeysTail* const tail = x.has_tail ? &x.tail : nullptr;
  int rc = CE_OK;
  if (n > 0 && lfu) {
    hipLaunchKernelGGL(k_slots_lfu, dim3(std::min(grid_for(n, 8192), kMaxBlocks)), dim3(1024), 0, s, slots_out, n,
                       c.inverted_cached_idx, c.freq_cnter, (const Ctl*)h->ctl);
    if (tail) {
      rc = tail->src_keys
               ? ce_bag_presort_window_src(slots_out, tail->nnz_per_batch, tail->n_batches, C, tail->lay.offsets,
                                           tail->lay.offsets_are_i64, tail->lay.offsets_batch_stride, tail->lay.num_bags,
                                           tail->lay.include_last_offset, tail->lay.hook_features, tail->keys_out, stream)
               : ce_bag_presort_window(slots_out, tail->nnz_per_batch, tail->n_batches, C, tail->keys_out, stream);
      if (rc) return rc;
    }
  } else if (n > 0 && tail) {
    rc = presort_window_from_rows(slots_out, tail->nnz_per_batch, tail->n_batches, C, c.inverted_cached_idx,
                                  &h->ctl->status, tail->src_keys, tail->lay, tail->keys_out, s);
    if (rc) return rc;
  } else if (n > 0) {
    hipLaunchKernelGGL(k_slots, dim3(grid_for(n, 256 * 4)), dim3(256), 0, s, slots_out, n, c.inverted_cached_idx,
                       (const Ctl*)h->ctl);
  }
  phase_mark(h);
  return CE_OK;
}


static int admit_parked(ce_cache* h) {
  const ce_cache::Pending& x = h->pend;
  const ce_cache_config_t& c = h->cfg;
  const Layout& L = h->L;
  const long long scap = (long long)L.stage_rows;
  CE_HIP_CHECK(hipStreamWaitValue64(x.s, h->wb->sig, (uint64_t)x.in_job, hipStreamWaitValueGte, ~0ull));
  const int ugrid = (int)std::min<int64_t>(1024, std::max<int64_t>(1, cdiv(L.stage_rows, 256 >> h->g_log2)));
  for_rows(h, [&](auto r) {
    using VT = typename decltype(r)::VT;
    hipLaunchKernelGGL((k_unpack_admitted<VT>), dim3(ugrid), dim3(256), 0, x.s, h->free_list,
                       (const long long*)&h->ctl->n_miss, scap, (const VT*)h->in_stage, (VT*)c.cache_weight, h->rowlen,
                       h->g_log2, h->ctl, (const unsigned long long*)(h->wb->sig_dev + 1), x.in_job,
                       (const int32_t*)h->miss_list,
                       L.list_cap > L.stage_rows ? (const VT*)c.host_weight_dev : (const VT*)nullptr);
  });
  return CE_OK;
}

static int admit_zero_copy(ce_cache* h) {
  const ce_cache::Pending& x = h->pend;
  const ce_cache_config_t& c = h->cfg;
  const long long scap = (long long)h->L.stage_rows;
  const int cap_groups = x.cap_groups;
  const int wb_groups = c.protect_depth > 0 ? std::max(1, cap_groups / 2) : cap_groups;
  auto swap = [&](auto r, auto rows) {
    using VT = typename decltype(r)::VT;
    hipLaunchKernelGGL((k_swap<VT, decltype(rows)::value>), dim3(wb_groups + cap_groups), dim3(x.swap_threads), 0, x.s,
                       h->stage_idx, (const VT*)h->stage, scap, wb_groups, h->miss_list, h->free_list,
                       (const long long*)&h->ctl->n_miss, (VT*)c.host_weight_dev, (VT*)c.cache_weight, h->rowlen,
                       h->g_log2, (const Ctl*)h->ctl);
  };
  if (h->vec && x.n <= 131072) swap(RowTag<f32x4>{}, std::integral_constant<int, 4>{});
  else for_rows(h, [&](auto r) { swap(r, std::integral_constant<int, 16>{}); });
  return CE_OK;
}

static int prepare_ids_second_half(ce_cache* h) {
  ce_cache::Pending& x = h->pend;
  if (x.chained) return chained_second_half(h);
  x.active = false;
  PhaseProf* const prof = live_prof(h);
  int rc = CE_OK;
  if (x.sel_pending) {
    x.sel_pending = false;
    if (prof) {
      (void)hipEventRecord(prof->resume[x.pslot], x.s);
      prof->resumed[x.pslot] = true;
    }
    rc = select_and_stage(h);
    if (rc) return rc;
  }
  const ce_cache_config_t& c = h->cfg;
  hipStream_t s = x.s;
  rc = x.worker ? admit_parked(h) : c.transport == CE_TRANSPORT_ZEROCOPY ? admit_zero_copy(h) : admit_staged(h);
  if (rc) return rc;
  hipLaunchKernelGGL(k_admit_maps, dim3(grid_for(h->L.list_cap, 256)), dim3(256), 0, s, h->miss_list, h->free_list,
                     (const long long*)&h->ctl->n_miss, 0ll, c.cached_idx_map, c.inverted_cached_idx,
                     c.freq_cnter, (const int64_t*)nullptr, h->slot_epoch, 0, h->ctl, h->ring_dev,
                     x.seq_arg, x.worker ? (const unsigned long long*)(h->wb->sig_dev + 1) : nullptr, x.in_job);
  phase_mark(h);
  rc = launch_slots_keys(h);
  if (rc) return rc;
  if (prof) prof->pending[x.pslot] = true;
  CE_LAUNCH_CHECK();
  if (!x.capturing) CE_HIP_CHECK(hipEventRecord(h->ev, s));
  return CE_OK;
}

extern "C" int ce_cache_prepare_ids(ce_cache_t* h, const int64_t* ids, int64_t n, int64_t* slots_out,
                                    ce_stream_t stream) {
  return prepare_ids_impl(h, ids, n, slots_out, stream, 0);
}

extern "C" int ce_cache_prepare_ids_keys(ce_cache_t* h, const int64_t* ids, int64_t n_batches, int64_t nnz_per_batch,
                                         int64_t* slots_out, int32_t src_keys, const void* offsets,
                                         int32_t offsets_are_i64, int64_t offsets_batch_stride, int64_t num_bags,
                                         int32_t include_last_offset, int64_t hook_features, uint64_t* keys_out,
                                         ce_stream_t stream) {
  CE_REQUIRE(n_batches > 0 && nnz_per_batch > 0 && keys_out, CE_ERR_INVALID, "bad window shape / null keys_out");
  KeysTail t{n_batches, nnz_per_batch, src_keys,
             {offsets, offsets_are_i64, offsets_batch_stride, num_bags, include_last_offset, hook_features}, keys_out};
  return prepare_ids_impl(h, ids, n_batches * nnz_per_batch, slots_out, stream, 0, &t);
}

extern "C" int ce_cache_prepare_ids_begin(ce_cache_t* h, const int64_t* ids, int64_t n_batches, int64_t nnz_per_batch,
                                          int64_t* slots_out, int32_t src_keys, const void* offsets,
                                          int32_t offsets_are_i64, int64_t offsets_batch_stride, int64_t num_bags,
                                          int32_t include_last_offset, int64_t hook_features, uint64_t* keys_out,
                                          ce_stream_t stream) {
  CE_REQUIRE(n_batches > 0 && nnz_per_batch > 0, CE_ERR_INVALID, "bad window shape");
  if (!keys_out) return prepare_ids_impl(h, ids, n_batches * nnz_per_batch, slots_out, stream, 0, nullptr, 1);
  KeysTail t{n_batches, nnz_per_batch, src_keys,
             {offsets, offsets_are_i64, offsets_batch_stride, num_bags, include_last_offset, hook_features}, keys_out};
  return prepare_ids_impl(h, ids, n_batches * nnz_per_batch, slots_out, stream, 0, &t, 1);
}

extern "C" int ce_cache_prepare_ids_finish(ce_cache_t* h, ce_stream_t stream) {
  CE_REQUIRE(h, CE_ERR_INVALID, "null handle");
  CE_REQUIRE(h->pend.active, CE_ERR_INVALID, "no cache op has been begun");
  CE_REQUIRE((hipStream_t)stream == h->pend.s, CE_ERR_INVALID, "finish the cache op on the stream it was begun on");
  return prepare_ids_second_half(h);
}

extern "C" int ce_cache_prepare_ids_padded(ce_cache_t* h, const int64_t* ids, int64_t n, int64_t* slots_out,
                                           ce_stream_t stream) {
  return prepare_ids_impl(h, ids, n, slots_out, stream, 1);
}

extern "C" int ce_cache_prepare_ids_begin_padded(ce_cache_t* h, const int64_t* ids, int64_t n, int64_t* slots_out,
                                                 ce_stream_t stream) {
// ... 47 lines not shown
    if (out) memset(out, 0, sizeof(*out));
    return CE_OK;
  }
  const ce_call_stats_t& r = h->history.back();
  if (out) *out = r;
  if (r.status == CE_ERR_CAPACITY)
    set_error("You move %lld embedding rows from CPU to CUDA. %lld rows are available on CUDA. "
              "Please increase cuda_row_num or decrease the training batch size.",
              (long long)r.n_unique, (long long)h->cfg.cuda_row_num);
  else if (r.status == CE_ERR_RANGE)
    set_error("an id is outside [0, %lld)", (long long)h->cfg.num_embeddings);
  return r.status;
}

extern "C" int ce_cache_totals(ce_cache_t* h, int64_t* cpu_to_cuda_numel, int64_t* cuda_to_cpu_numel,
                               int64_t* cache_miss, int64_t* total_cache, int64_t* n_calls) {
  CE_REQUIRE(h, CE_ERR_INVALID, "null handle");
  drain(h);
  if (cpu_to_cuda_numel) *cpu_to_cuda_numel = h->cpu_to_cuda_numel;
  if (cuda_to_cpu_numel) *cuda_to_cpu_numel = h->cuda_to_cpu_numel;
  if (cache_miss) *cache_miss = h->cache_miss;
  if (total_cache) *total_cache = h->total_cache;
  if (n_calls) *n_calls = h->drained;
  return CE_OK;
}

extern "C" int ce_cache_failures(ce_cache_t* h, int64_t* n_failed, int32_t* last_status, int64_t* last_seq) {
  CE_REQUIRE(h, CE_ERR_INVALID, "null handle");
  drain(h);
  if (n_failed) *n_failed = h->n_failed;
  if (last_status) *last_status = h->last_fail_status;
  if (last_seq) *last_seq = h->last_fail_seq;
  return CE_OK;
}

extern "C" int64_t ce_cache_history(ce_cache_t* h, int64_t first_seq, ce_call_stats_t* out, int64_t cap) {
  if (!h || !out || cap <= 0) return 0;
  drain(h);
  if (h->history.empty()) return 0;
  int64_t i = first_seq - h->hist_base;
  if (i < 0) i = 0;
  int64_t w = 0;
  for (; i < (int64_t)h->history.size() && w < cap; ++i) out[w++] = h->history[(size_t)i];
  return w;
}

extern "C" int ce_cache_lookup_slots(ce_cache_t* h, const int64_t* ids, int64_t n, int64_t* slots_out,
                                     ce_stream_t stream) {
  CE_REQUIRE(h, CE_ERR_INVALID, "null handle");
  if (n == 0) return CE_OK;
  CE_REQUIRE(ids && slots_out && n > 0, CE_ERR_INVALID, "null ids/slots");
  const ce_cache_config_t& c = h->cfg;
  hipLaunchKernelGGL(k_lookup, dim3(grid_for(n, 256)), dim3(256), 0, (hipStream_t)stream, ids, n, c.idx_map,
                     c.inverted_cached_idx, c.num_embeddings, slots_out);
  CE_LAUNCH_CHECK();
  return CE_OK;
}

extern "C" int ce_cache_flush(ce_cache_t* h, ce_stream_t stream) {
  CE_REQUIRE(h, CE_ERR_INVALID, "null handle");
  CE_REQUIRE(!h->pend.active, CE_ERR_INVALID, "a cache op begun with ce_cache_prepare_ids_begin has not been finished");
  int rc = before_call(h);
  if (rc) return rc;
  hipStream_t s = (hipStream_t)stream;
  const ce_cache_config_t& c = h->cfg;
  const int64_t C = c.cuda_row_num;
  if (h->wb) {
    rc = h->wb->wait_out(h->wb->out_issued);
    if (rc) return rc;
  }
  rc = join_rows(h, s);
  if (rc) return rc;
  h->seq += 1;
  h->free_zero = false;
  h->free_reset_seq = h->seq;
  const int gpb = 256 >> h->g_log2;
  hipLaunchKernelGGL(k_begin, dim3(1), dim3(256), 0, s, h->ctl, (int32_t*)nullptr, 0, (uint32_t*)nullptr,
                     (long long)h->seq);
  for_rows(h, [&](auto r) {
    using VT = typename decltype(r)::VT;
    hipLaunchKernelGGL((k_flush_rows<VT>), dim3(grid_for(C, gpb)), dim3(256), 0, s, c.cached_idx_map, C,
                       (const VT*)c.cache_weight, (VT*)c.host_weight_dev, h->rowlen, h->g_log2);
  });
  hipLaunchKernelGGL(k_flush_maps, dim3(grid_for(C, 256)), dim3(256), 0, s, c.cached_idx_map, C,
                     c.inverted_cached_idx, c.freq_cnter, h->slot_epoch, h->ctl);
  hipLaunchKernelGGL(k_flush_end, dim3(1), dim3(1), 0, s, C, h->ctl, h->ring_dev + (h->seq % kRing),
                     (long long)h->seq);
  CE_LAUNCH_CHECK();
  CE_HIP_CHECK(hipEventRecord(h->ev, s));
  return CE_OK;
}

extern "C" int ce_cache_set_protect_depth(ce_cache_t* h, int32_t depth) {
  CE_REQUIRE(h && depth >= 0 && depth < 1024, CE_ERR_INVALID, "bad protect depth");
  h->cfg.protect_depth = depth;
  return CE_OK;
}

extern "C" int ce_cache_set_buffer_rows(ce_cache_t* h, int64_t rows) {
  CE_REQUIRE(h && rows >= 0, CE_ERR_INVALID, "bad buffer_rows");
  h->buffer_rows = rows;
  return CE_OK;
}

extern "C" int ce_cache_set_transport(ce_cache_t* h, int32_t transport) {
  CE_REQUIRE(h && (transport == CE_TRANSPORT_ZEROCOPY || transport == CE_TRANSPORT_STAGED ||
                   transport == CE_TRANSPORT_WORKER), CE_ERR_INVALID, "bad transport");
  if (h->cfg.transport == transport) return CE_OK;
  CE_REQUIRE(!h->pend.active, CE_ERR_INVALID, "a cache op begun with ce_cache_prepare_ids_begin has not been finished");
  if (h->wb) {
    int rc = h->wb->wait_out(h->wb->out_issued);
    if (rc == CE_OK) rc = h->wb->wait_in(h->wb->in_issued);
    if (rc) return rc;
    CE_HIP_CHECK(hipEventSynchronize(h->ev));
    if (hipEvent_t ev = last_rows_event(h)) CE_HIP_CHECK(hipEventSynchronize(ev));
    h->wb->probe_floor = h->wb->out_issued + 1;
  }
  h->cfg.transport = transport;
  if (transport == CE_TRANSPORT_WORKER) return ensure_writeback(h);
  return CE_OK;
}

extern "C" int32_t ce_cache_get_transport(ce_cache_t* h) { return h ? h->cfg.transport : -1; }

extern "C" int ce_cache_set_cache_weight(ce_cache_t* h, float* cache_weight) {
  CE_REQUIRE(h && cache_weight, CE_ERR_INVALID, "null handle / pointer");
  CE_REQUIRE(!h->vec || ((uintptr_t)cache_weight & 15) == 0, CE_ERR_INVALID, "the cache must keep its 16-byte alignment");
  CE_HIP_CHECK(hipDeviceSynchronize());
  h->cfg.cache_weight = cache_weight;
  return CE_OK;
}

extern "C" int ce_cache_set_profiling(ce_cache_t* h, int32_t on) {
  CE_REQUIRE(h, CE_ERR_INVALID, "null handle");
  if (on && !h->prof) h->prof = new PhaseProf();
  if (!on && h->prof) {
    for (int i = 0; i < kProfDepth; ++i) h->prof->collect(i);
    delete h->prof;
// ... 53 lines not shown
```

cachedembedding_amd/csrc/ce_cache_fused.h:

```cpp
#pragma once

namespace ce {

constexpr unsigned long long kLbAggregate = 1ull, kLbPrefix = 2ull;
__device__ __forceinline__ unsigned long long lb_pack(unsigned tag, unsigned long long state, unsigned a, unsigned b) {
  return ((unsigned long long)(tag & 0xffffu) << 48) | (state << 46) | ((unsigned long long)(a & 0x7fffffu) << 23) |
         (unsigned long long)(b & 0x7fffffu);
}
__device__ __forceinline__ void lb_scan_wave(unsigned long long* words, int j, unsigned tag, unsigned a, unsigned b,
                                             unsigned* base_a, unsigned* base_b) {
  const int lane = threadIdx.x & 63;
  unsigned sa = 0, sb = 0;
  if (j > 0) {
    if (lane == 0)
      __hip_atomic_store(&words[j], lb_pack(tag, kLbAggregate, a, b), __ATOMIC_RELAXED, __HIP_MEMORY_SCOPE_AGENT);
    const unsigned long long t0 = wall_clock64();
    int i = j - 1;
    bool done = false;
    while (!done) {
      unsigned long long w[4];
#pragma unroll
      for (int q = 0; q < 4; ++q) {
        const int idx = i - 64 * q - lane;
        w[q] = idx >= 0 ? __hip_atomic_load(&words[idx], __ATOMIC_RELAXED, __HIP_MEMORY_SCOPE_AGENT)
                        : lb_pack(tag, kLbPrefix, 0u, 0u);
      }
      bool again = false;
#pragma unroll
      for (int q = 0; q < 4; ++q) {
        if (done || again) continue;
        const unsigned long long st = (w[q] >> 46) & 3ull;
        const bool valid = (unsigned)(w[q] >> 48) == (tag & 0xffffu) && st != 0;
        const unsigned long long m_inv = __ballot(!valid), m_pre = __ballot(valid && st == kLbPrefix);
        const unsigned long long m_stop = m_inv | m_pre;
        const int stop = m_stop ? __ffsll((long long)m_stop) - 1 : 64;
        const bool stop_is_prefix = m_stop && ((m_pre >> stop) & 1ull);
        const bool take = lane < stop || (lane == stop && stop_is_prefix);
        unsigned xa = take ? (unsigned)(w[q] >> 23) & 0x7fffffu : 0u, xb = take ? (unsigned)w[q] & 0x7fffffu : 0u;
#pragma unroll
        for (int d = 32; d >= 1; d >>= 1) {
          xa += __shfl_xor(xa, d);
          xb += __shfl_xor(xb, d);
        }
        sa += xa;
        sb += xb;
        if (stop_is_prefix) {
          done = true;
        } else if (m_stop) {
          i = i - 64 * q - stop;
          again = true;
        }
      }
      if (!done && !again) i -= 256;
      if (again) {
        __builtin_amdgcn_s_sleep(1);
        if (wall_clock64() - t0 > 400000000ull) __builtin_trap();
      }
    }
  }
  if (lane == 0)
    __hip_atomic_store(&words[j], lb_pack(tag, kLbPrefix, sa + a, sb + b), __ATOMIC_RELAXED, __HIP_MEMORY_SCOPE_AGENT);
  *base_a = sa;
  *base_b = sb;
}


template <int U>
__global__ __launch_bounds__(1024) void k_touch(const int64_t* __restrict__ ids, int64_t n,
                                               const int32_t* __restrict__ idx_map,
                                               const int32_t* __restrict__ inverted, int64_t N, uint32_t* bitmap,
                                               int32_t* fine, int32_t* coarse, int32_t* slot_epoch, long long seq_arg,
                                               FrontWords* fw, int32_t* miss_tmp, unsigned miss_cap, int64_t* rows_out,
                                               int allow_pad) {
  __shared__ int wcnt[16], wcold[16];
  __shared__ unsigned base_s;
  const int lane = threadIdx.x & 63, wv = threadIdx.x >> 6, nw = (int)blockDim.x >> 6;
  const int32_t epoch = call_epoch(seq_arg);
  const int64_t i0 = ((int64_t)blockIdx.x * blockDim.x + (threadIdx.x & ~63)) * U;
  int32_t row[U], inv[U];
  bool valid[U], first[U];
  bool bad = false;
#pragma unroll
  for (int u = 0; u < U; ++u) {
    const int64_t i = i0 + u * 64 + lane;
    valid[u] = i < n;
    row[u] = 0;
    if (valid[u]) {
      const int64_t id = ids[i];
      if ((unsigned long long)id >= (unsigned long long)N) {
        if (!(allow_pad && id == -1)) bad = true;
        valid[u] = false;
        rows_out[i] = -1;
      } else {
        row[u] = idx_map ? idx_map[id] : (int32_t)id;
      }
    }
  }
#pragma unroll
  for (int u = 0; u < U; ++u) {
    inv[u] = 0;
    if (valid[u]) {
      rows_out[i0 + u * 64 + lane] = row[u];
      inv[u] = inverted[row[u]];
    }
  }
  int cold = 0, mine = 0;
#pragma unroll
  for (int u = 0; u < U; ++u) {
    first[u] = false;
    if (!valid[u]) continue;
    if (inv[u] >= 0) {
      slot_epoch[inv[u]] = epoch;
    } else {
      ++cold;
      const uint32_t bit = 1u << (row[u] & 31);
      const uint32_t old = atomicOr(bitmap + (row[u] >> 5), bit);
      first[u] = (old & bit) == 0;
      mine += first[u] ? 1 : 0;
    }
  }
  const int winc = wave_incl_scan(mine, lane);
  cold = wave_sum(cold);
  if (lane == 63) wcnt[wv] = winc;
  if (lane == 0) wcold[wv] = cold;
  __syncthreads();
  if (threadIdx.x == 0) {
    int tot = 0, tc = 0;
    for (int k = 0; k < nw; ++k) {
      tot += wcnt[k];
      tc += wcold[k];
    }
    base_s = tot ? atomicAdd(&fw->n_miss, (unsigned)tot) : 0u;
    if (tc) atomicAdd(&fw->miss_lookups, (unsigned long long)tc);
  }
  __syncthreads();
  unsigned pos = base_s + (unsigned)(winc - mine);
  for (int k = 0; k < wv; ++k) pos += (unsigned)wcnt[k];
#pragma unroll
  for (int u = 0; u < U; ++u) {
    if (!first[u]) continue;
    if (pos < miss_cap) miss_tmp[pos] = row[u];
    ++pos;
    atomicAdd(fine + (row[u] >> kFineShift), 1);
    atomicAdd(coarse + (row[u] >> kChunkShift), 1);
  }
  if (bad) fw->bad = 1;
}

__global__ __launch_bounds__(256) void k_front_cleanup(const int32_t* __restrict__ miss_tmp, const FrontWords* fw,
                                                       uint32_t* bitmap, int32_t* fine, int32_t* coarse, int n_chunks) {
  front_cleanup(miss_tmp, fw, bitmap, fine, coarse, n_chunks);
}

__global__ __launch_bounds__(256) void k_miss_rank(const int32_t* __restrict__ miss_tmp, FrontWords* fw,
                                                   FrontWords* fw_next, const uint32_t* __restrict__ bitmap,
                                                   const int32_t* __restrict__ fine,
                                                   const int32_t* __restrict__ coarse, int n_chunks,
                                                   unsigned miss_cap, int32_t* miss_list,
                                                   const int32_t* __restrict__ slot_epoch,
                                                   int64_t C, uint32_t* hist, long long seq_arg, Ctl* ctl,
                                                   int64_t n_ids, ce_call_stats_t* ring, long long in_cap,
                                                   int assume_free0, long long* n_admit_out) {
  extern __shared__ int cbase[];
// ... 72 lines not shown
    const int tot = wtot[0] + wtot[1] + wtot[2] + wtot[3];
    if (tot) __hip_atomic_fetch_add(&fw->hit_unique, (unsigned)tot, __ATOMIC_RELAXED, __HIP_MEMORY_SCOPE_AGENT);
    const unsigned ticket = __hip_atomic_fetch_add(&fw->done, 1u, __ATOMIC_ACQ_REL, __HIP_MEMORY_SCOPE_AGENT);
    last_s = ticket == gridDim.x - 1;
    if (last_s) {
      const long long hu = __hip_atomic_load(&fw->hit_unique, __ATOMIC_RELAXED, __HIP_MEMORY_SCOPE_AGENT);
      ce_call_stats_t* const ring_slot = ring + (seq_arg % kRing);
      const long long free0 = ctl->n_free;
      const long long tu = hu + m_all;
      int status = fw->bad ? CE_ERR_RANGE : CE_OK;
      if (status == CE_OK && (tu > C || m_all > miss_cap)) status = CE_ERR_CAPACITY;
      if (status == CE_OK && assume_free0 && free0 != 0) status = CE_ERR_HIP;
      const long long tm = status == CE_OK ? (long long)m : 0;
      if (m_all > miss_cap) fw->overflow = 1;
      long long k = 0;
      if (status == CE_OK) {
        k = tm - free0;
        if (k < 0) k = 0;
        ctl->n_free = free0 + k - tm;
      }
      ctl->seq = seq_arg;
      ctl->n_free_start = free0;
      ctl->n_unique = tu;
      ctl->n_miss = tm;
      ctl->k_evict = k;
      ctl->sel_krem = k;
      ctl->sel_prefix = 0;
      ctl->miss_lookups = (long long)fw->miss_lookups;
      ctl->n_eligible = 0;
      ctl->victims_count = 0;
      ctl->lost = 0;
      __hip_atomic_store(&ctl->status, status, __ATOMIC_RELAXED, __HIP_MEMORY_SCOPE_AGENT);
      ring_slot->n_ids = n_ids;
      ring_slot->n_unique = tu;
      ring_slot->n_miss = tm;
      ring_slot->n_evict = k;
      ring_slot->miss_lookups = (status == CE_OK) ? (long long)fw->miss_lookups : 0;
      ring_slot->n_free_after = ctl->n_free;
      ring_slot->status = status;
      ring_slot->kind = CE_CALL_PREPARE;
      if (n_admit_out) *n_admit_out = tm < in_cap ? tm : in_cap;
      fw_next->miss_lookups = 0;
      fw_next->n_miss = 0;
      fw_next->hit_unique = 0;
      fw_next->done = 0;
      fw_next->bad = 0;
      fw_next->overflow = 0;
    }
  }
}

struct StageArgs {
  int32_t* cached_idx_map;
  int32_t* inverted;
  int64_t* freq;
  int32_t* slot_epoch;
  int64_t C;
  long long seq_arg;
  int top_pass;
  const unsigned long long* keys;
  const uint32_t* hist;
  Ctl* ctl;
  unsigned long long* lb;
  unsigned tag;
  int32_t* free_list;
  const int32_t* miss_list;
  ce_call_stats_t* ring;
  long long* n_unpack_out;
  const void* cache;
  void* stage;
  int32_t* stage_rows_idx;
  long long scap;
  int rowlen, g_log2, vec;
  WbMail* mail;
  long long job;
  EvTable evt;
  void* host_overflow;
};

constexpr int kRemapSlots = 4096;

__global__ __launch_bounds__(256) void k_rank_victims(const StageArgs a) {
  __shared__ unsigned long long prefix_s;
  __shared__ int fail_s, go_s;
  __shared__ unsigned long long mask_s[64];
  __shared__ int pre_s[65];
  __shared__ unsigned base_s;
  Ctl* const ctl = a.ctl;
  const int lane = threadIdx.x & 63, wv = threadIdx.x >> 6;
  const int j = (int)blockIdx.x;
  const int64_t s0 = (int64_t)j * kRemapSlots;
  unsigned long long key[16];
#pragma unroll
  for (int u = 0; u < 16; ++u) {
    const int64_t sl = s0 + (int64_t)(wv + 4 * u) * 64 + lane;
    key[u] = sl < a.C ? a.keys[sl] : ~0ull;
  }
  if (threadIdx.x < 64) {
    const SelState st = select_level(a.hist, 0, a.top_pass, ctl, threadIdx.x, false);
    if (threadIdx.x == 0) {
      prefix_s = st.prefix;
      fail_s = st.fail;
      go_s = (ctl->k_evict != 0 && ctl->status == CE_OK) ? 1 : 0;
    }
  }
  __syncthreads();
  if (!go_s) return;
// ... 18 lines not shown
  }
  __syncthreads();
  if (threadIdx.x < 64) {
    const int cgrp = __popcll(mask_s[threadIdx.x]);
    const int inc = wave_incl_scan(cgrp, lane);
    pre_s[threadIdx.x] = inc - cgrp;
    unsigned b0 = 0, b1 = 0;
    lb_scan_wave(a.lb, j, a.tag, (unsigned)__shfl(inc, 63), 0u, &b0, &b1);
    if (threadIdx.x == 0) base_s = b0;
  }
  __syncthreads();
  const long long base = base_s;
  const unsigned long long lt = lane == 0 ? 0ull : (~0ull >> (64 - lane));
#pragma unroll
  for (int u = 0; u < 16; ++u) {
    const int g = wv + 4 * u;
    const unsigned long long mk = mask_s[g];
    if ((mk >> lane) & 1) {
      const long long pos = base + pre_s[g] + __popcll(mk & lt);
      if (pos < k) a.free_list[pos] = (int32_t)(s0 + (int64_t)g * 64 + lane);
    }
  }
}

template <typename VT>
__device__ __forceinline__ void stage_and_remap(const StageArgs& a, long long k, int32_t epoch) {
  const VT* const cache = (const VT*)a.cache;
  VT* const stage = (VT*)a.stage;
  VT* const host = (VT*)a.host_overflow;
  const int rowlen = a.rowlen;
  const int Gl = 1 << a.g_log2;
  const int gl = threadIdx.x & (Gl - 1);
  const long long gstride = ((long long)gridDim.x * blockDim.x) >> a.g_log2;
  constexpr int R = kStageRowsInFlight;
  for (long long i0 = ((((long long)blockIdx.x * blockDim.x + threadIdx.x)) >> a.g_log2) * R; i0 < k; i0 += gstride * R) {
    int32_t slot[R], old[R], in_row[R];
    VT v[R];
#pragma unroll
    for (int t = 0; t < R; ++t) {
      slot[t] = i0 + t < k ? a.free_list[i0 + t] : -1;
      in_row[t] = (i0 + t < k && gl == 0) ? a.miss_list[i0 + t] : -1;
    }
#pragma unroll
    for (int t = 0; t < R; ++t) {
      old[t] = (slot[t] >= 0 && gl == 0) ? a.cached_idx_map[slot[t]] : -1;
      if (slot[t] >= 0 && rowlen <= Gl && gl < rowlen) v[t] = cache[(int64_t)slot[t] * rowlen + gl];
    }
#pragma unroll
    for (int t = 0; t < R; ++t) {
      if (slot[t] < 0) continue;
      const long long i = i0 + t;
      const bool staged = i < a.scap;
      if (gl == 0) {
        a.inverted[old[t]] = -1;
        a.cached_idx_map[slot[t]] = in_row[t];
        a.inverted[in_row[t]] = slot[t];
        a.slot_epoch[slot[t]] = epoch;
        if (a.freq) a.freq[slot[t]] = 0;
        if (staged) {
          a.stage_rows_idx[i] = old[t];
          if (a.evt.keys) evt_insert(a.evt, (uint32_t)a.job, old[t], (int32_t)i);
        }
      }
      int32_t row = 0;
      if (!staged) row = __shfl(old[t], (threadIdx.x & 63) & ~(Gl - 1));
      if (rowlen <= Gl) {
        if (gl < rowlen) {
          if (staged) stage[i * rowlen + gl] = v[t];
          else if (host) host[(int64_t)row * rowlen + gl] = v[t];
        }
      } else {
        VT* const dst = staged ? stage + i * rowlen : (host ? host + (int64_t)row * rowlen : nullptr);
        if (dst) copy_row(cache + (int64_t)slot[t] * rowlen, dst, rowlen, gl, Gl);
      }
    }
  }
}

__global__ __launch_bounds__(256) void k_stage_maps(const StageArgs a) {
  Ctl* const ctl = a.ctl;
  const long long seq = call_seq(ctl, a.seq_arg);
  const int32_t epoch = call_epoch(seq);
  const long long k = (ctl->status == CE_OK) ? ctl->k_evict : 0;
  if (blockIdx.x == 0 && threadIdx.x == 0) {
    ce_call_stats_t* const ring_slot = a.ring + (seq % kRing);
    *a.n_unpack_out = k;
    if (a.mail) {
      a.mail->count = k < a.scap ? k : a.scap;
      a.mail->job = a.job;
    }
    __threadfence_system();
    *(volatile long long*)&ring_slot->seq = seq;
  }
  if (a.vec) stage_and_remap<f32x4>(a, k, epoch);
  else stage_and_remap<float>(a, k, epoch);
}

template <typename VT>
__global__ __launch_bounds__(256) void k_unpack_chained(const int32_t* __restrict__ slots, const long long* n_ptr,
                                                        long long cap, const VT* __restrict__ in_stage, VT* cache,
                                                        int rowlen, int g_log2, const int32_t* __restrict__ rows,
                                                        const VT* __restrict__ host,
                                                        const unsigned long long* __restrict__ evt_keys,
                                                        const int32_t* __restrict__ evt_pos, uint32_t evt_mask,
                                                        uint32_t tag, const VT* __restrict__ prev_stage) {
  const long long n_all = *n_ptr;
  const int G = 1 << g_log2;
  const int gl = threadIdx.x & (G - 1);
  const int64_t gstride = ((int64_t)gridDim.x * blockDim.x) >> g_log2;
// ... 31 lines not shown
```

cachedembedding_amd/csrc/ce_cache_rows.h:

```cpp
#pragma once

namespace ce {

template <typename VT>
__device__ __forceinline__ void copy_row(const VT* __restrict__ src, VT* __restrict__ dst, int rowlen, int gl, int G) {
  for (int c = gl; c < rowlen; c += G) dst[c] = src[c];
}

constexpr int kSwapRows = 16;

template <typename VT>
__global__ __launch_bounds__(1024) void k_evict(const int32_t* __restrict__ victims, int32_t* cached_idx_map,
                                               int32_t* inverted, const VT* __restrict__ cache, VT* host,
                                               long long first, int rowlen, int g_log2, const Ctl* ctl) {
  const long long k = (ctl->status == CE_OK) ? ctl->k_evict : 0;
  if (k <= first) return;
  const int G = 1 << g_log2;
  const int gl = threadIdx.x & (G - 1);
  const int64_t gstride = ((int64_t)gridDim.x * blockDim.x) >> g_log2;
  if (!host) return;
  for (int64_t i = first + (((int64_t)blockIdx.x * blockDim.x + threadIdx.x) >> g_log2) * kSwapRows; i < k;
       i += gstride * kSwapRows) {
    if (rowlen <= G) {
      VT v[kSwapRows];
      int64_t dst[kSwapRows];
#pragma unroll
      for (int t = 0; t < kSwapRows; ++t) {
        dst[t] = -1;
        if (i + t < k) {
          const int32_t slot = victims[i + t];
          dst[t] = cached_idx_map[slot];
          if (gl < rowlen) v[t] = cache[(int64_t)slot * rowlen + gl];
        }
      }
#pragma unroll
      for (int t = 0; t < kSwapRows; ++t) {
        if (dst[t] < 0) continue;
        if (gl < rowlen) host[dst[t] * rowlen + gl] = v[t];
        if (gl == 0) {
          inverted[dst[t]] = -1;
          cached_idx_map[victims[i + t]] = -1;
        }
      }
    } else {
      for (int t = 0; t < kSwapRows && i + t < k; ++t) {
        const int32_t slot = victims[i + t];
        const int32_t row = cached_idx_map[slot];
        copy_row(cache + (int64_t)slot * rowlen, host + (int64_t)row * rowlen, rowlen, gl, G);
        __builtin_amdgcn_wave_barrier();
        if (gl == 0) {
          inverted[row] = -1;
          cached_idx_map[slot] = -1;
        }
      }
    }
  }
}
constexpr int kStageRowsInFlight = 4;

__device__ __forceinline__ void free_list_from_victims(const unsigned long long* __restrict__ keys, int64_t C,
                                                       const int32_t* __restrict__ blk_vic, int32_t* free_list,
                                                       const Ctl* ctl, int j) {
  if (ctl->status != CE_OK || ctl->k_evict == 0) return;
  const unsigned long long T = ctl->sel_prefix_after[0];
  const long long need = ctl->n_miss;
  __shared__ int part_s[4];
  __shared__ unsigned long long mask_s[64];
  __shared__ int pre_s[65];
  const int lane = threadIdx.x & 63, wv = threadIdx.x >> 6;
  int part = 0;
  for (int i = threadIdx.x; i < j; i += 256) part += blk_vic[i];
  part = wave_sum(part);
  if (lane == 0) part_s[wv] = part;
  const int64_t s0 = (int64_t)j * 4096;
#pragma unroll
  for (int u = 0; u < 16; ++u) {
    const int g = wv + 4 * u;
    const int64_t sl = s0 + (int64_t)g * 64 + lane;
    const unsigned long long key = sl < C ? keys[sl] : ~0ull;
    const unsigned long long m = __ballot(key <= T && key != ~0ull);
    if (lane == 0) mask_s[g] = m;
  }
  __syncthreads();
  if (threadIdx.x < 64) {
    const int c = __popcll(mask_s[threadIdx.x]);
    const int inc = wave_incl_scan(c, lane);
    pre_s[threadIdx.x] = inc - c;
  }
  __syncthreads();
  const long long base = (long long)part_s[0] + part_s[1] + part_s[2] + part_s[3];
  const unsigned long long lt = lane == 0 ? 0ull : (~0ull >> (64 - lane));
#pragma unroll
  for (int u = 0; u < 16; ++u) {
    const int g = wv + 4 * u;
    const unsigned long long m = mask_s[g];
    if ((m >> lane) & 1) {
      const long long pos = base + pre_s[g] + __popcll(m & lt);
      if (pos < need) free_list[pos] = (int32_t)(s0 + (int64_t)g * 64 + lane);
    }
  }
}

struct EvTable {
  unsigned long long* keys;
  int32_t* pos;
  uint32_t mask;
};
__device__ __forceinline__ uint32_t evt_hash(int32_t row, uint32_t mask) {
  return (((uint32_t)row * 2654435761u) >> 7) & mask;
}
__device__ __forceinline__ void evt_insert(const EvTable t, uint32_t tag, int32_t row, int32_t pos) {
  const unsigned long long mine = ((unsigned long long)tag << 32) | (uint32_t)row;
  uint32_t h = evt_hash(row, t.mask);
  for (;;) {
    const unsigned long long cur = __hip_atomic_load(&t.keys[h], __ATOMIC_RELAXED, __HIP_MEMORY_SCOPE_AGENT);
    if ((uint32_t)(cur >> 32) == tag) {
      h = (h + 1) & t.mask;
      continue;
    }
    if (atomicCAS(&t.keys[h], cur, mine) == cur) {
      t.pos[h] = pos;
      return;
    }
  }
}
__device__ __forceinline__ int32_t evt_find(const unsigned long long* __restrict__ keys,
                                            const int32_t* __restrict__ pos, uint32_t mask, uint32_t tag,
                                            int32_t row) {
  uint32_t h = evt_hash(row, mask);
  for (;;) {
    const unsigned long long cur = keys[h];
    if ((uint32_t)(cur >> 32) != tag) return -1;
    if ((uint32_t)cur == (uint32_t)row) return pos[h];
    h = (h + 1) & mask;
  }
}

template <typename VT>
__global__ __launch_bounds__(256) void k_evict_stage(const int32_t* __restrict__ victims,
                                                     int32_t* cached_idx_map, int32_t* inverted,
                                                     const VT* __restrict__ cache, VT* stage, int32_t* stage_rows_idx,
                                                     long long cap, int rowlen, int g_log2, const Ctl* ctl,
                                                     WbMail* mail, long long job, int stage_grid,
                                                     const unsigned long long* __restrict__ keys, int64_t C,
                                                     const int32_t* __restrict__ blk_vic, int32_t* free_list,
                                                     EvTable evt, VT* host_overflow) {
  if ((int)blockIdx.x >= stage_grid) {
    free_list_from_victims(keys, C, blk_vic, free_list, ctl, (int)blockIdx.x - stage_grid);
    return;
  }
  const long long k_all = (ctl->status == CE_OK) ? ctl->k_evict : 0;
  long long k = k_all;
  if (k > cap) k = cap;
  if (host_overflow && k_all > cap) {
    const int G0 = 1 << g_log2;
    const int gl0 = threadIdx.x & (G0 - 1);
    const int64_t gs0 = ((int64_t)stage_grid * blockDim.x) >> g_log2;
    for (int64_t i = cap + (((int64_t)blockIdx.x * blockDim.x + threadIdx.x) >> g_log2); i < k_all; i += gs0) {
      const int32_t slot = victims[i];
      const int32_t row = cached_idx_map[slot];
      if (row < 0) continue;
      copy_row(cache + (int64_t)slot * rowlen, host_overflow + (int64_t)row * rowlen, rowlen, gl0, G0);
      __builtin_amdgcn_wave_barrier();
      if (gl0 == 0) {
        inverted[row] = -1;
        cached_idx_map[slot] = -1;
      }
    }
  }
  if (mail && blockIdx.x == 0 && threadIdx.x == 0) {
    mail->count = k;
    mail->job = job;
  }
  const int G = 1 << g_log2;
  const int gl = threadIdx.x & (G - 1);
  const int64_t gstride = ((int64_t)stage_grid * blockDim.x) >> g_log2;
  constexpr int R = kStageRowsInFlight;
  for (int64_t i = (((int64_t)blockIdx.x * blockDim.x + threadIdx.x) >> g_log2) * R; i < k; i += gstride * R) {
    if (rowlen <= G) {
      int32_t slot[R];
      VT v[R];
#pragma unroll
      for (int t = 0; t < R; ++t) slot[t] = i + t < k ? victims[i + t] : -1;
#pragma unroll
      for (int t = 0; t < R; ++t) {
        if (slot[t] < 0) continue;
        if (gl == 0) {
          const int32_t row = cached_idx_map[slot[t]];
          stage_rows_idx[i + t] = row;
          inverted[row] = -1;
          cached_idx_map[slot[t]] = -1;
          if (evt.keys) evt_insert(evt, (uint32_t)job, row, (int32_t)(i + t));
        }
        if (gl < rowlen) v[t] = cache[(int64_t)slot[t] * rowlen + gl];
      }
#pragma unroll
      for (int t = 0; t < R; ++t)
        if (slot[t] >= 0 && gl < rowlen) stage[(i + t) * rowlen + gl] = v[t];
    } else {
      for (int t = 0; t < R && i + t < k; ++t) {
        const int32_t slot = victims[i + t];
        if (gl == 0) {
          const int32_t row = cached_idx_map[slot];
          stage_rows_idx[i + t] = row;
          inverted[row] = -1;
          cached_idx_map[slot] = -1;
          if (evt.keys) evt_insert(evt, (uint32_t)job, row, (int32_t)(i + t));
        }
        copy_row(cache + (int64_t)slot * rowlen, stage + (i + t) * rowlen, rowlen, gl, G);
      }
    }
  }
}

template <typename VT, int R>
__device__ __forceinline__ void writeback_rows(const int32_t* __restrict__ stage_rows_idx,
                                               const VT* __restrict__ stage, VT* host, long long cap, int rowlen,
                                               int g_log2, const Ctl* ctl, int block, int nblocks) {
  long long k = (ctl->status == CE_OK) ? ctl->k_evict : 0;
  if (k > cap) k = cap;
  const int G = 1 << g_log2;
  const int gl = threadIdx.x & (G - 1);
  const int64_t gstride = ((int64_t)nblocks * blockDim.x) >> g_log2;
  for (int64_t i = (((int64_t)block * blockDim.x + threadIdx.x) >> g_log2) * R; i < k;
       i += gstride * R) {
    if (rowlen <= G) {
      VT v[R];
      int64_t dst[R];
#pragma unroll
      for (int t = 0; t < R; ++t) {
        dst[t] = -1;
        if (i + t < k) {
          dst[t] = stage_rows_idx[i + t];
          if (gl < rowlen) v[t] = stage[(i + t) * rowlen + gl];
        }
      }
#pragma unroll
      for (int t = 0; t < R; ++t)
        if (dst[t] >= 0 && gl < rowlen) host[dst[t] * rowlen + gl] = v[t];
    } else {
      for (int t = 0; t < R && i + t < k; ++t)
        copy_row(stage + (i + t) * rowlen, host + (int64_t)stage_rows_idx[i + t] * rowlen, rowlen, gl, G);
    }
  }
}

__global__ __launch_bounds__(256) void k_evict_maps(const int32_t* __restrict__ victims, int32_t* cached_idx_map,
                                                    int32_t* inverted, int32_t* evicted_rows, const Ctl* ctl) {
  const long long k = (ctl->status == CE_OK) ? ctl->k_evict : 0;
  const int64_t stride = (int64_t)gridDim.x * blockDim.x;
  for (int64_t i = (int64_t)blockIdx.x * blockDim.x + threadIdx.x; i < k; i += stride) {
    const int32_t slot = victims[i];
    const int32_t row = cached_idx_map[slot];
    if (evicted_rows) evicted_rows[i] = row;
    inverted[row] = -1;
    cached_idx_map[slot] = -1;
  }
}

__global__ __launch_bounds__(256) void k_free_count(const int32_t* __restrict__ cached_idx_map, int64_t C,
                                                    int32_t* blk_free, const Ctl* ctl) {
  if (ctl->status != CE_OK || ctl->n_miss == 0) return;
  const int64_t s0 = ((int64_t)blockIdx.x * 256 + threadIdx.x) * 4;
  int f = 0;
#pragma unroll
  for (int t = 0; t < 4; ++t)
    if (s0 + t < C) f += (cached_idx_map[s0 + t] < 0);
  __shared__ int sf[4];
  f = wave_sum(f);
  if ((threadIdx.x & 63) == 0) sf[threadIdx.x >> 6] = f;
  __syncthreads();
  if (threadIdx.x == 0) blk_free[blockIdx.x] = sf[0] + sf[1] + sf[2] + sf[3];
}

__global__ __launch_bounds__(256) void k_free_emit(const int32_t* __restrict__ cached_idx_map, int64_t C,
                                                   const int32_t* __restrict__ blk_free, int32_t* free_list,
                                                   const Ctl* ctl) {
  if (ctl->status != CE_OK || ctl->n_miss == 0) return;
  const long long need = ctl->n_miss;
  __shared__ int wsum4[4];
  int part = 0;
  for (int i = threadIdx.x; i < (int)blockIdx.x; i += 256) part += blk_free[i];
  part = wave_sum(part);
  if ((threadIdx.x & 63) == 0) wsum4[threadIdx.x >> 6] = part;
  __syncthreads();
  const long long before = (long long)wsum4[0] + wsum4[1] + wsum4[2] + wsum4[3];
  if (before >= need) return;
  const int64_t s0 = ((int64_t)blockIdx.x * 256 + threadIdx.x) * 4;
  int fl[4];
  int f = 0;
#pragma unroll
  for (int t = 0; t < 4; ++t) {
    fl[t] = (s0 + t < C) && (cached_idx_map[s0 + t] < 0);
    f += fl[t];
  }
  int tot;
  long long pos = block_excl_scan_256(f, &tot) + before;
#pragma unroll
  for (int t = 0; t < 4; ++t) {
    if (fl[t]) {
      if (pos < need) free_list[pos] = (int32_t)(s0 + t);
      ++pos;
    }
  }
}

__global__ __launch_bounds__(1024) void k_free_single(const int32_t* __restrict__ cached_idx_map, int64_t C,
                                                      int32_t* free_list, const Ctl* ctl) {
// ... 123 lines not shown
                                                         int rowlen, int g_log2, Ctl* ctl,
                                                         const unsigned long long* fail_word, long long job,
                                                         const int32_t* __restrict__ rows,
                                                         const VT* __restrict__ host_overflow) {
  const bool ok = ctl->status == CE_OK;
  if (blockIdx.x == 0 && threadIdx.x == 0) {
    ctl->lost = *(volatile const unsigned long long*)fail_word == (unsigned long long)job;
  }
  if (!ok) return;
  long long n = *n_ptr;
  const int G = 1 << g_log2;
  const int gl = threadIdx.x & (G - 1);
  const int64_t gstride = ((int64_t)gridDim.x * blockDim.x) >> g_log2;
  if (host_overflow && n > cap) {
    for (int64_t i = cap + (((int64_t)blockIdx.x * blockDim.x + threadIdx.x) >> g_log2); i < n; i += gstride)
      copy_row(host_overflow + (int64_t)rows[i] * rowlen, cache + (int64_t)slots[i] * rowlen, rowlen, gl, G);
  }
  if (n > cap) n = cap;
  constexpr int R = kStageRowsInFlight;
  for (int64_t i = (((int64_t)blockIdx.x * blockDim.x + threadIdx.x) >> g_log2) * R; i < n; i += gstride * R) {
    if (rowlen <= G) {
      int32_t slot[R];
      VT v[R];
#pragma unroll
      for (int t = 0; t < R; ++t) {
        slot[t] = i + t < n ? slots[i + t] : -1;
        if (slot[t] >= 0 && gl < rowlen) v[t] = in_stage[(i + t) * rowlen + gl];
      }
#pragma unroll
      for (int t = 0; t < R; ++t)
        if (slot[t] >= 0 && gl < rowlen) cache[(int64_t)slot[t] * rowlen + gl] = v[t];
    } else {
      for (int t = 0; t < R && i + t < n; ++t)
        copy_row(in_stage + (i + t) * rowlen, cache + (int64_t)slots[i + t] * rowlen, rowlen, gl, G);
    }
  }
}

template <typename VT, int R>
__global__ __launch_bounds__(1024) void k_swap(const int32_t* __restrict__ stage_rows_idx,
                                              const VT* __restrict__ stage, long long cap, int wb_blocks,
                                              const int32_t* __restrict__ rows, const int32_t* __restrict__ slots,
                                              const long long* n_ptr, VT* host, VT* cache, int rowlen, int g_log2,
                                              const Ctl* ctl) {
  if ((int)blockIdx.x < wb_blocks)
    writeback_rows<VT, R>(stage_rows_idx, stage, host, cap, rowlen, g_log2, ctl, (int)blockIdx.x, wb_blocks);
  else
    admit_rows<VT, R>(rows, slots, n_ptr, 0ll, (const VT*)host, cache, rowlen, g_log2, ctl,
                      (int)blockIdx.x - wb_blocks, (int)gridDim.x - wb_blocks);
}

__global__ __launch_bounds__(256) void k_admit_maps(const int32_t* __restrict__ rows,
                                                    const int32_t* __restrict__ slots, const long long* n_ptr,
                                                    long long n_imm, int32_t* cached_idx_map, int32_t* inverted,
                                                    int64_t* freq, const int64_t* freq_vals, int32_t* slot_epoch,
                                                    int32_t epoch_imm, Ctl* ctl, ce_call_stats_t* ring,
                                                    long long seq_arg, const unsigned long long* fail_word,
                                                    long long job, long long* n_unpack_out = nullptr) {
  const long long seq = ring ? call_seq(ctl, seq_arg) : 0;
  const int32_t epoch = ring ? call_epoch(seq) : epoch_imm;
  ce_call_stats_t* const ring_slot = ring ? ring + (seq % kRing) : nullptr;
  const bool lost = fail_word && ctl->lost != 0;
  if (ring_slot && blockIdx.x == 0 && threadIdx.x == 0) {
    if (n_unpack_out) *n_unpack_out = (ctl->status == CE_OK && n_ptr) ? *n_ptr : 0;
    if (lost && ctl->status == CE_OK) {
      ctl->n_free = ctl->n_free + ctl->n_miss;
      ring_slot->status = CE_ERR_HIP;
      ring_slot->n_free_after = ctl->n_free;
      __hip_atomic_store(&ctl->status, CE_ERR_HIP, __ATOMIC_RELAXED, __HIP_MEMORY_SCOPE_AGENT);
    }
    __threadfence_system();
    *(volatile long long*)&ring_slot->seq = seq;
  }
  if (lost) return;
  if (ctl && __hip_atomic_load(&ctl->status, __ATOMIC_RELAXED, __HIP_MEMORY_SCOPE_AGENT) != CE_OK) return;
  const long long n = n_ptr ? *n_ptr : n_imm;
  const int64_t stride = (int64_t)gridDim.x * blockDim.x;
  for (int64_t i = (int64_t)blockIdx.x * blockDim.x + threadIdx.x; i < n; i += stride) {
    const int32_t row = rows ? rows[i] : (int32_t)i;
    const int32_t slot = slots ? slots[i] : (int32_t)i;
    cached_idx_map[slot] = row;
    inverted[row] = slot;
    if (freq) freq[slot] = freq_vals ? freq_vals[i] : 0;
    slot_epoch[slot] = epoch;
  }
}

__global__ __launch_bounds__(256) void k_lookup(const int64_t* __restrict__ ids, int64_t n,
                                                const int32_t* __restrict__ idx_map,
                                                const int32_t* __restrict__ inverted, int64_t N, int64_t* slots_out) {
  const int64_t stride = (int64_t)gridDim.x * blockDim.x;
  for (int64_t i = (int64_t)blockIdx.x * blockDim.x + threadIdx.x; i < n; i += stride) {
    const int64_t id = ids[i];
    int64_t slot = -1;
    if ((unsigned long long)id < (unsigned long long)N) slot = inverted[idx_map ? idx_map[id] : (int32_t)id];
    slots_out[i] = slot;
  }
}

__global__ __launch_bounds__(256) void k_slots(int64_t* slots, int64_t n, const int32_t* __restrict__ inverted,
                                               const Ctl* ctl) {
  const bool failed = ctl->status != CE_OK;
  constexpr int U = 4;
  const int64_t stride = (int64_t)gridDim.x * blockDim.x * U;
  for (int64_t i0 = (int64_t)blockIdx.x * blockDim.x * U + threadIdx.x; i0 < n; i0 += stride) {
    int64_t row[U];
#pragma unroll
    for (int u = 0; u < U; ++u) {
      const int64_t i = i0 + (int64_t)u * blockDim.x;
      row[u] = i < n ? slots[i] : -1;
    }
#pragma unroll
    for (int u = 0; u < U; ++u) {
      const int64_t i = i0 + (int64_t)u * blockDim.x;
      if (i < n) slots[i] = (failed || row[u] < 0) ? -1 : (int64_t)inverted[row[u]];
    }
  }
}

constexpr int kSlotsHashBits = 13;
constexpr int kSlotsHash = 1 << kSlotsHashBits;
__global__ __launch_bounds__(1024) void k_slots_lfu(int64_t* slots, int64_t n, const int32_t* __restrict__ inverted,
                                                    int64_t* freq, const Ctl* ctl) {
  __shared__ int hkey[kSlotsHash];
  __shared__ int hcnt[kSlotsHash];
  for (int i = threadIdx.x; i < kSlotsHash; i += blockDim.x) { hkey[i] = -1; hcnt[i] = 0; }
  __syncthreads();
  const bool failed = ctl->status != CE_OK;
  const int64_t per_block = (n + gridDim.x - 1) / gridDim.x;
  const int64_t lo = (int64_t)blockIdx.x * per_block;
  const int64_t hi = lo + per_block < n ? lo + per_block : n;
  constexpr int U = 4;
  for (int64_t i0 = lo + threadIdx.x; i0 < hi; i0 += (int64_t)blockDim.x * U) {
    int64_t row[U];
    int slot[U];
#pragma unroll
    for (int u = 0; u < U; ++u) {
      const int64_t i = i0 + (int64_t)u * blockDim.x;
      row[u] = (i < hi && !failed) ? slots[i] : -1;
    }
#pragma unroll
    for (int u = 0; u < U; ++u) slot[u] = row[u] >= 0 ? inverted[row[u]] : -1;
#pragma unroll
    for (int u = 0; u < U; ++u) {
      const int64_t i = i0 + (int64_t)u * blockDim.x;
      if (i < hi) slots[i] = slot[u];
      if (slot[u] < 0) continue;
      unsigned h = ((unsigned)slot[u] * 2654435761u) >> (32 - kSlotsHashBits);
      bool done = false;
      for (int p = 0; p < 16 && !done; ++p) {
        const int old = atomicCAS(&hkey[h], -1, slot[u]);
        if (old == -1 || old == slot[u]) {
          atomicAdd(&hcnt[h], 1);
          done = true;
        } else {
          h = (h + 1) & (kSlotsHash - 1);
        }
      }
      if (!done) atomicAdd((unsigned long long*)&freq[slot[u]], 1ull);
    }
  }
  __syncthreads();
  for (int i = threadIdx.x; i < kSlotsHash; i += blockDim.x)
    if (hkey[i] >= 0) atomicAdd((unsigned long long*)&freq[hkey[i]], (unsigned long long)hcnt[i]);
}

template <typename VT>
__global__ __launch_bounds__(256) void k_flush_rows(const int32_t* __restrict__ cached_idx_map, int64_t C,
                                                    const VT* __restrict__ cache, VT* host, int rowlen,
                                                    int g_log2) {
  const int G = 1 << g_log2;
  const int gl = threadIdx.x & (G - 1);
  const int64_t gstride = ((int64_t)gridDim.x * blockDim.x) >> g_log2;
  for (int64_t s = ((int64_t)blockIdx.x * blockDim.x + threadIdx.x) >> g_log2; s < C; s += gstride) {
    const int32_t row = cached_idx_map[s];
    if (row >= 0) copy_row(cache + s * rowlen, host + (int64_t)row * rowlen, rowlen, gl, G);
  }
}

__global__ __launch_bounds__(256) void k_flush_maps(int32_t* cached_idx_map, int64_t C, int32_t* inverted,
                                                    int64_t* freq, int32_t* slot_epoch, Ctl* ctl) {
  const int64_t stride = (int64_t)gridDim.x * blockDim.x;
  int n = 0;
  for (int64_t s = (int64_t)blockIdx.x * blockDim.x + threadIdx.x; s < C; s += stride) {
    const int32_t row = cached_idx_map[s];
    if (row >= 0) {
      inverted[row] = -1;
      cached_idx_map[s] = -1;
      ++n;
    }
    if (freq) freq[s] = INT64_MAX;
    slot_epoch[s] = kEpochNever;
  }
  n = wave_sum(n);
  if ((threadIdx.x & 63) == 0 && n) atomicAdd((unsigned long long*)&ctl->k_evict, (unsigned long long)n);
}

__global__ void k_flush_end(int64_t C, Ctl* ctl, ce_call_stats_t* ring_slot, long long seq) {
  ctl->seq = seq;
  ctl->n_free = C;
  ring_slot->n_ids = 0;
  ring_slot->n_unique = 0;
  ring_slot->n_miss = 0;
  ring_slot->n_evict = ctl->k_evict;
  ring_slot->miss_lookups = 0;
  ring_slot->n_free_after = C;
  ring_slot->status = CE_OK;
  ring_slot->kind = CE_CALL_FLUSH;
  __threadfence_system();
  ring_slot->seq = seq;
}

__global__ void k_preload_end(long long n, Ctl* ctl, ce_call_stats_t* ring_slot, long long seq) {
  ctl->seq = seq;
  ctl->n_free -= n;
  ring_slot->n_ids = 0;
  ring_slot->n_unique = n;
  ring_slot->n_miss = n;
  ring_slot->n_evict = 0;
  ring_slot->miss_lookups = 0;
  ring_slot->n_free_after = ctl->n_free;
  ring_slot->status = CE_OK;
  ring_slot->kind = CE_CALL_PRELOAD;
  __threadfence_system();
  ring_slot->seq = seq;
}

__global__ __launch_bounds__(256) void k_fill_i32(int32_t* p, int64_t n, int32_t v) {
  const int64_t stride = (int64_t)gridDim.x * blockDim.x;
  for (int64_t i = (int64_t)blockIdx.x * blockDim.x + threadIdx.x; i < n; i += stride) p[i] = v;
}
__global__ __launch_bounds__(256) void k_fill_i64(int64_t* p, int64_t n, int64_t v) {
  const int64_t stride = (int64_t)gridDim.x * blockDim.x;
  for (int64_t i = (int64_t)blockIdx.x * blockDim.x + threadIdx.x; i < n; i += stride) p[i] = v;
}

template <typename VT>
__global__ __launch_bounds__(256) void k_pack_rows(const int32_t* __restrict__ slots, long long n,
                                                   const VT* __restrict__ cache, VT* staging, int rowlen,
                                                   int g_log2) {
// ... 19 lines not shown
```

cachedembedding_amd/csrc/ce_common.h:

```cpp
#pragma once
#include <hip/hip_runtime.h>
#include <sched.h>
#include <stdint.h>
#include <stdio.h>
#include <string.h>

#include <type_traits>

#include "ce_api.h"

namespace ce {

void set_error(const char* fmt, ...);

#define CE_HIP_CHECK(expr)                                                              \
  do {                                                                                  \
    hipError_t _e = (expr);                                                             \
    if (_e != hipSuccess) {                                                             \
      ce::set_error("%s failed: %s (%s:%d)", #expr, hipGetErrorString(_e), __FILE__, __LINE__); \
      return CE_ERR_HIP;                                                                \
    }                                                                                   \
  } while (0)

#define CE_REQUIRE(cond, code, ...)  \
// ... 8 lines not shown

typedef float f32x4 __attribute__((ext_vector_type(4)));

template <typename VT> __device__ __forceinline__ VT vzero();
template <> __device__ __forceinline__ float vzero<float>() { return 0.f; }
template <> __device__ __forceinline__ f32x4 vzero<f32x4>() { return f32x4{0.f, 0.f, 0.f, 0.f}; }

typedef __bf16 bf16_t;
typedef _Float16 f16_t;
typedef bf16_t bf16x4 __attribute__((ext_vector_type(4)));
typedef f16_t f16x4 __attribute__((ext_vector_type(4)));

template <typename AT, typename VT> struct Act;
template <typename VT> struct Act<float, VT> {
  typedef VT V;
  static __device__ __forceinline__ VT up(V a) { return a; }
  static __device__ __forceinline__ V down(VT v) { return v; }
};
#define CE_ACT16(AT, AT4)                                                                                     \
  template <> struct Act<AT, float> {                                                                         \
    typedef AT V;                                                                                             \
    static __device__ __forceinline__ float up(V a) { return (float)a; }                                      \
    static __device__ __forceinline__ V down(float v) { return (AT)v; }                                       \
  };                                                                                                          \
  template <> struct Act<AT, f32x4> {                                                                         \
    typedef AT4 V;                                                                                            \
    static __device__ __forceinline__ f32x4 up(V a) { return __builtin_convertvector(a, f32x4); }             \
    static __device__ __forceinline__ V down(f32x4 v) { return __builtin_convertvector(v, AT4); }             \
  };
CE_ACT16(bf16_t, bf16x4)
CE_ACT16(f16_t, f16x4)
#undef CE_ACT16

static inline int64_t cdiv(int64_t a, int64_t b) { return (a + b - 1) / b; }

constexpr int kNumCU = 256;
constexpr int kMaxBlocks = kNumCU * 8;

static inline int grid_for(int64_t work_items, int per_block) {
  int64_t b = cdiv(work_items, per_block);
  if (b < 1) b = 1;
  if (b > kMaxBlocks) b = kMaxBlocks;
  return (int)b;
}

struct BagLayout {
  const void* offsets;
  int32_t offsets_are_i64;
  int64_t offsets_batch_stride, num_bags;
  int32_t include_last_offset;
  int64_t hook_features;
};

int presort_window_from_rows(int64_t* slots_io, int64_t nnz_per_batch, int64_t n_batches, int64_t num_rows,
                             const int32_t* inverted, const int* status, int32_t src_keys, const BagLayout& lay,
                             uint64_t* keys_out, hipStream_t stream);

void bind_thread_near_gpu();
bool near_gpu_cpus(cpu_set_t* out);

struct SortedRows {
  const int32_t* rows;
  const int32_t* lookups;
  const int32_t* bag_of;
};
size_t sorted_rows_bytes(int64_t nnz);
int sorted_rows(const int64_t* indices, int64_t nnz, int64_t num_rows, const void* offsets, int off64,
                int64_t num_bags, int include_last, void* workspace, hipStream_t s,
                SortedRows& out);

struct RowGeom {
  bool vec;
  int rowlen;
  int g_log2;
  int nch;
};

static inline int row_geometry(int32_t dim, bool aligned, RowGeom& r) {
  r.vec = dim % 4 == 0 && aligned;
  r.rowlen = r.vec ? dim / 4 : dim;
  int g = 1;
  r.g_log2 = 0;
  while (g < r.rowlen && g < 64) { g <<= 1; ++r.g_log2; }
  const int need = (r.rowlen - 1) / g + 1;
  r.nch = 1;
  while (r.nch < need) r.nch <<= 1;
  CE_REQUIRE(r.nch <= 4, CE_ERR_UNSUPPORTED, "embedding dim %d too large for this build", dim);
  return CE_OK;
}

static inline bool al16(const void* q) { return (((uintptr_t)q) & 15) == 0; }
static inline bool act_aligned(const void* q, int act) { return (((uintptr_t)q) & (act == CE_ACT_F32 ? 15 : 7)) == 0; }

#define CE_REQUIRE_ROWS(num_rows) \
  CE_REQUIRE((num_rows) > 0 && (num_rows) < (int64_t)INT32_MAX, CE_ERR_INVALID, "num_rows out of range")

#define CE_REQUIRE_ACT(act)                                                                            \
  CE_REQUIRE((act) == CE_ACT_F32 || (act) == CE_ACT_BF16 || (act) == CE_ACT_F16, CE_ERR_INVALID,       \
             "unknown activation dtype %d (CE_ACT_F32 / CE_ACT_BF16 / CE_ACT_F16)", (int)(act))

static inline int w16_check(int32_t weight_dtype, int32_t dim) {
  CE_REQUIRE(weight_dtype == CE_ACT_BF16 || weight_dtype == CE_ACT_F16, CE_ERR_INVALID,
             "weight_dtype %d: a 16-bit table is CE_ACT_BF16 or CE_ACT_F16", (int)weight_dtype);
  CE_REQUIRE(dim > 0, CE_ERR_INVALID, "embedding dim must be positive");
  CE_REQUIRE(dim % 8 == 0 && dim <= 1024, CE_ERR_UNSUPPORTED,
             "a 16-bit table needs dim %% 8 == 0 and dim <= 1024 (got %d)", (int)dim);
  return CE_OK;
}

// ... 34 lines not shown
```

include/ce_api.h:

```cpp
#ifndef CE_API_H
#define CE_API_H

#include <stddef.h>
#include <stdint.h>

#ifdef __cplusplus
extern "C" {
#endif

#define CE_API_VERSION 6

#define CE_OK 0
#define CE_ERR_INVALID 1
#define CE_ERR_HIP 2
#define CE_ERR_CAPACITY 3
#define CE_ERR_NOMEM 4
#define CE_ERR_UNSUPPORTED 5
#define CE_ERR_RANGE 6

#define CE_EVICT_DATASET 0
#define CE_EVICT_LFU 1
#define CE_EVICT_LRU 2

#define CE_MODE_SUM 0
// ... 269 lines not shown
  int64_t n_unique;
  int64_t n_miss;
  int64_t n_evict;
  int64_t miss_lookups;
  int64_t n_free_after;
  int32_t status;
  int32_t kind;
} ce_call_stats_t;

#define CE_CALL_PREPARE 0
#define CE_CALL_PRELOAD 1
#define CE_CALL_FLUSH 2

size_t ce_cache_workspace_bytes(int64_t num_embeddings, int64_t cuda_row_num, int64_t max_ids_per_call,
                                int32_t embedding_dim);

int ce_cache_create(const ce_cache_config_t* cfg, ce_stream_t stream, ce_cache_t** out);
int ce_cache_destroy(ce_cache_t* h);

int ce_cache_preload(ce_cache_t* h, const int32_t* rows, const int64_t* freq_vals, int64_t n,
                     ce_stream_t stream);

int ce_cache_set_freq_bound(ce_cache_t* h, int64_t bound);

int ce_cache_prepare_ids(ce_cache_t* h, const int64_t* ids, int64_t n, int64_t* slots_out,
                         ce_stream_t stream);
int ce_cache_prepare_ids_keys(ce_cache_t* h, const int64_t* ids, int64_t n_batches, int64_t nnz_per_batch,
                              int64_t* slots_out, int32_t src_keys, const void* offsets, int32_t offsets_are_i64,
                              int64_t offsets_batch_stride, int64_t num_bags, int32_t include_last_offset,
                              int64_t hook_features, uint64_t* keys_out, ce_stream_t stream);
int ce_cache_prepare_ids_begin(ce_cache_t* h, const int64_t* ids, int64_t n_batches, int64_t nnz_per_batch,
                               int64_t* slots_out, int32_t src_keys, const void* offsets, int32_t offsets_are_i64,
                               int64_t offsets_batch_stride, int64_t num_bags, int32_t include_last_offset,
                               int64_t hook_features, uint64_t* keys_out, ce_stream_t stream);
int ce_cache_prepare_ids_finish(ce_cache_t* h, ce_stream_t stream);
int ce_cache_prepare_ids_padded(ce_cache_t* h, const int64_t* ids, int64_t n, int64_t* slots_out,
                                ce_stream_t stream);
int ce_cache_prepare_ids_begin_padded(ce_cache_t* h, const int64_t* ids, int64_t n, int64_t* slots_out,
                                      ce_stream_t stream);

int ce_cache_set_deferred_rows(ce_cache_t* h, int32_t on);
int64_t ce_cache_rows_ticket(ce_cache_t* h);
int ce_cache_wait_rows(ce_cache_t* h, int64_t ticket, ce_stream_t stream);

int ce_cache_last_stats(ce_cache_t* h, ce_call_stats_t* out);
int ce_cache_totals(ce_cache_t* h, int64_t* cpu_to_cuda_numel, int64_t* cuda_to_cpu_numel,
                    int64_t* cache_miss, int64_t* total_cache, int64_t* n_calls);
int ce_cache_failures(ce_cache_t* h, int64_t* n_failed, int32_t* last_status, int64_t* last_seq);
int64_t ce_cache_history(ce_cache_t* h, int64_t first_seq, ce_call_stats_t* out, int64_t cap);

int ce_cache_lookup_slots(ce_cache_t* h, const int64_t* ids, int64_t n, int64_t* slots_out,
                          ce_stream_t stream);

int ce_cache_flush(ce_cache_t* h, ce_stream_t stream);

int ce_cache_set_protect_depth(ce_cache_t* h, int32_t depth);
int ce_cache_set_transport(ce_cache_t* h, int32_t transport);
int32_t ce_cache_get_transport(ce_cache_t* h);
int ce_cache_set_cache_weight(ce_cache_t* h, float* cache_weight);
int ce_cache_graph_replayed(ce_cache_t* h, int64_t n_calls, int64_t ids_per_call, ce_stream_t stream);
int ce_cache_set_profiling(ce_cache_t* h, int32_t on);
int32_t ce_cache_phase_count(void);
const char* ce_cache_phase_name(int32_t i);
int ce_cache_phase_times(ce_cache_t* h, double* ms_out, int32_t cap, int64_t* calls, int32_t reset);
int ce_cache_writeback_wait(ce_cache_t* h);
int ce_cache_swap_stats(ce_cache_t* h, double* seconds6, int64_t* counts4);
int ce_cache_set_buffer_rows(ce_cache_t* h, int64_t rows);
int ce_cache_free_rows(ce_cache_t* h, int64_t* out);

size_t ce_bucketize_workspace(int64_t n, int32_t world);
int ce_bucketize_rows(const int64_t* ids, int64_t n, const int32_t* idx_map, int32_t world,
                      int64_t* local_rows_out, int64_t* perm_out, int64_t* counts_out,
                      void* workspace, size_t workspace_bytes, ce_stream_t stream);

int ce_dedupe_bucket_rows(const int64_t* ids, int64_t n, const int32_t* idx_map, int64_t num_rows,
                          int32_t world, int32_t* stamp, int32_t* slot_of_row, int32_t* scratch,
                          int64_t* local_rows_out, int64_t* pos_out, int64_t* counts_out, ce_stream_t stream);

int ce_dedupe_bucket_rows_padded(const int64_t* ids, int64_t n, const int32_t* idx_map, int64_t num_rows,
                                 int32_t world, int64_t capacity, int32_t* stamp, int32_t* slot_of_row,
                                 int32_t* scratch, int64_t* local_rows_out, int64_t* pos_out, int64_t* counts_out,
                                 int32_t* overflow_flag, ce_stream_t stream);

int ce_dedupe_bucket_rows_padded_window(const int64_t* ids, int64_t n, int64_t n_batches, const int32_t* idx_map,
                                        int64_t num_rows, int32_t world, int64_t capacity, int32_t* stamp,
                                        int32_t* slot_of_row, int32_t* scratch, int64_t* local_rows_out,
                                        int64_t* pos_out, int64_t* counts_out, int32_t* overflow_flag,
                                        ce_stream_t stream);

int ce_exchange_local_index(const int64_t* pos, int64_t n_per_batch, int64_t n_batches, const int64_t* slots,
                            int64_t slots_batch_stride, int64_t local_lo, int64_t local_hi, int64_t tail_base,
                            int64_t* index_out, ce_stream_t stream);

int ce_split_classify(const int64_t* serve, int32_t world, int32_t n_batches, int64_t capacity, int64_t n_local_rows,
                      const int64_t* prev, int64_t n_prev, uint64_t* mask, uint8_t* flags_out, ce_stream_t stream);

int ce_split_places(const int64_t* ids, const uint8_t* flags, int32_t n_batches, int32_t world, int64_t capacity,
                    int32_t skip_peer, const int32_t* caps, int32_t* place_fwd, int32_t* place_bwd,
                    int32_t* counts_out, int32_t* overflow_flag, ce_stream_t stream);

int ce_exchange_local_index_split(const int64_t* pos, int64_t n_per_batch, int64_t n_batches, const int64_t* slots,
                                  const int32_t* place_fwd, const int32_t* place_bwd, int64_t chunk_stride,
                                  int64_t local_lo, int64_t local_hi, int64_t tail_base, int64_t bwd_base,
                                  const int32_t* caps, int32_t world, int64_t n_early, int64_t n_urgent,
                                  int64_t n_deferred, int64_t* index_fwd, int64_t* index_bwd, ce_stream_t stream);

// ... 21 lines not shown
```

Measured before the change: 3.203 billion.

## Maintain a direct id-to-slot map to skip the idx_map/inverted indirection

Adds an optional id_slot array (with its reverse row_id), kept current wherever inverted_cached_idx is updated (admit, evict, flush), so the touch kernel can resolve an id's cache slot with one load instead of idx_map followed by inverted. Hits are written to the slot stream already resolved, and misses are encoded as negative row values; the slots, LFU-slots and presort kernels get an ENC variant that decodes them. The cost is two extra N-sized int32 arrays and extra scattered writes on every admit and evict. Graph-capture interaction is also restricted. It is on by default whenever an idx_map exists.

```diff
diff --git a/cachedembedding_amd/_lib.py b/cachedembedding_amd/_lib.py
--- a/cachedembedding_amd/_lib.py
+++ b/cachedembedding_amd/_lib.py
@@ -182,6 +182,8 @@
                                 POINTER(c_int64), POINTER(c_int64)]),
     "ce_cache_history": (c_int64, [c_void_p, c_int64, POINTER(CeCallStats), c_int64]),
     "ce_cache_lookup_slots": (c_int, [c_void_p, c_void_p, c_int64, c_void_p, c_void_p]),
+    "ce_cache_set_id_slot_map": (c_int, [c_void_p, c_void_p, c_void_p, c_void_p]),
+    "ce_cache_has_id_slot_map": (c_int32, [c_void_p]),
     "ce_cache_flush": (c_int, [c_void_p, c_void_p]),
     "ce_cache_set_protect_depth": (c_int, [c_void_p, c_int32]),
     "ce_cache_set_transport": (c_int, [c_void_p, c_int32]),
diff --git a/cachedembedding_amd/cache_mgr.py b/cachedembedding_amd/cache_mgr.py
--- a/cachedembedding_amd/cache_mgr.py
+++ b/cachedembedding_amd/cache_mgr.py
@@ -176,6 +176,8 @@
             self.register_buffer("freq_cnter", torch.empty(C, device=dev, dtype=torch.int64), persistent=False)
         else:
             self.freq_cnter = None
+        self.id_slot: Optional[torch.Tensor] = None
+        self.row_id: Optional[torch.Tensor] = None
         self._max_ids = 2 ** 31 - 2
         self._deferred_rows = False
         self._handle = None
@@ -224,6 +226,30 @@
             check(lib.ce_cache_set_buffer_rows(h, int(self.buffer_size)))
         if reapply_worker:
             self.set_transport("worker")
+        self.sync_id_slot_map()
+
+    def sync_id_slot_map(self, enable: Optional[bool] = None) -> bool:
+        import os
+        if self._idx_map is None or self._handle is None:
+            return False
+        if enable is None:
+            if os.environ.get("CE_ID_SLOT_MAP", "1") == "0":
+                return False
+            enable = True
+        with torch.cuda.device(self.device):
+            if not enable:
+                check(lib.ce_cache_set_id_slot_map(self._handle, None, None, stream_ptr()))
+                return False
+            if self.id_slot is None:
+                N = self.num_embeddings
+                self.id_slot = torch.empty(N, device=self.device, dtype=torch.int32)
+                self.row_id = torch.empty(N, device=self.device, dtype=torch.int32)
+            check(lib.ce_cache_set_id_slot_map(self._handle, ptr(self.id_slot), ptr(self.row_id), stream_ptr()))
+        return True
+
+    @property
+    def has_id_slot_map(self) -> bool:
+        return bool(lib.ce_cache_has_id_slot_map(self._handle))
 
     @property
     def weight(self) -> torch.Tensor:
@@ -273,6 +299,7 @@
                 if fvals is not None:
                     check(lib.ce_cache_set_freq_bound(self._handle, int(fvals.max().item())))
                 torch.cuda.current_stream().synchronize()
+        self.sync_id_slot_map()
 
     def _recreate_with_idx_map(self):
         assert self.cuda_available_row_num == self.cuda_row_num, "reorder() after rows were cached"
diff --git a/cachedembedding_amd/cached_embedding.py b/cachedembedding_amd/cached_embedding.py
--- a/cachedembedding_amd/cached_embedding.py
+++ b/cachedembedding_amd/cached_embedding.py
@@ -117,6 +117,7 @@
                                                use_idx_map=True if _idx_map is not None else None)
         if _idx_map is not None:
             self.cache_weight_mgr._idx_map.copy_(_idx_map)
+            self.cache_weight_mgr.sync_id_slot_map()
         self.cache_weight_mgr.reorder(ids_freq_mapping, warmup_ratio)
         if q8:
             self.eval()
diff --git a/cachedembedding_amd/csrc/ce_bag.hip b/cachedembedding_amd/csrc/ce_bag.hip
--- a/cachedembedding_amd/csrc/ce_bag.hip
+++ b/cachedembedding_amd/csrc/ce_bag.hip
@@ -449,7 +449,7 @@
 constexpr int kExclRun = 32;
 constexpr unsigned kExclFlag = 0x80000000u;
 
-template <bool SRC, bool EXCL, bool ROWS>
+template <bool SRC, bool EXCL, int ROWS>
 __global__ __launch_bounds__(1024) void k_bag_presort_seg(const int64_t* __restrict__ indices, int64_t nnz_per_batch,
                                                          int32_t segs_per_batch, int64_t n_segs, uint32_t num_rows,
                                                          unsigned long long* __restrict__ keys_out, BagParams lay,
@@ -485,7 +485,7 @@
         row_r[r] = e < n_here ? (int32_t)slots_io[in_base + e] : -1;
       }
 #pragma unroll
-      for (int r = 0; r < kSegKeys; ++r) slot_r[r] = (row_r[r] >= 0 && !failed) ? inverted[row_r[r]] : -1;
+      for (int r = 0; r < kSegKeys; ++r) slot_r[r] = failed ? -1 : front_slot<ROWS == 2>((int64_t)row_r[r], inverted);
 #pragma unroll
       for (int r = 0; r < kSegKeys; ++r) {
         const int e = r * 1024 + tid;
@@ -1529,7 +1529,8 @@
 
 static int launch_presort(const int64_t* indices, int64_t* slots_io, const int32_t* inverted, const int* status,
                           int64_t nnz_per_batch, int64_t n_batches, int64_t num_rows, const BagLayout* L,
-                          const int64_t* ids, int64_t* ids_minmax, uint64_t* keys_out, hipStream_t s) {
+                          const int64_t* ids, int64_t* ids_minmax, uint64_t* keys_out, hipStream_t s,
+                          bool encoded = false) {
   if (nnz_per_batch == 0 || n_batches == 0) return CE_OK;
   CE_REQUIRE((slots_io ? inverted && status : indices != nullptr) && keys_out && nnz_per_batch > 0 && n_batches > 0,
              CE_ERR_INVALID, "bad arguments");
@@ -1552,11 +1553,16 @@
   };
   const std::true_type yes{};
   const std::false_type no{};
-  if (slots_io && L) launch(yes, no, yes);
-  else if (slots_io) launch(no, no, yes);
-  else if (L && ids_minmax) launch(yes, yes, no);
-  else if (L) launch(yes, no, no);
-  else launch(no, no, no);
+  const std::integral_constant<int, 0> slots{};
+  const std::integral_constant<int, 1> rows{};
+  const std::integral_constant<int, 2> enc{};
+  if (slots_io && L && encoded) launch(yes, no, enc);
+  else if (slots_io && L) launch(yes, no, rows);
+  else if (slots_io && encoded) launch(no, no, enc);
+  else if (slots_io) launch(no, no, rows);
+  else if (L && ids_minmax) launch(yes, yes, slots);
+  else if (L) launch(yes, no, slots);
+  else launch(no, no, slots);
   CE_LAUNCH_CHECK();
   return CE_OK;
 }
@@ -1564,9 +1570,9 @@
 namespace ce {
 int presort_window_from_rows(int64_t* slots_io, int64_t nnz_per_batch, int64_t n_batches, int64_t num_rows,
                              const int32_t* inverted, const int* status, int32_t src_keys, const BagLayout& lay,
-                             uint64_t* keys_out, hipStream_t stream) {
+                             uint64_t* keys_out, hipStream_t stream, bool encoded) {
   return launch_presort(nullptr, slots_io, inverted, status, nnz_per_batch, n_batches, num_rows, src_keys ? &lay : nullptr,
-                        nullptr, nullptr, keys_out, stream);
+                        nullptr, nullptr, keys_out, stream, encoded);
 }
 }
 
diff --git a/cachedembedding_amd/csrc/ce_cache.hip b/cachedembedding_amd/csrc/ce_cache.hip
--- a/cachedembedding_amd/csrc/ce_cache.hip
+++ b/cachedembedding_amd/csrc/ce_cache.hip
@@ -86,6 +86,8 @@
   bool free_zero = false;
   long long free_reset_seq = 0;
   bool deferred_rows = false;
+  int32_t *id_slot = nullptr, *row_id = nullptr;
+  bool captured_plain = false;
   struct Pending {
     bool active = false;
     int64_t n = 0;
@@ -93,6 +95,7 @@
     hipStream_t s = nullptr;
     bool worker = false, capturing = false, has_tail = false;
     bool chained = false;
+    bool enc = false;
     long long call = 0;
     int parity = 0;
     long long in_job = 0, seq_arg = 0;
@@ -113,6 +116,8 @@
 template <typename F> static inline void for_rows(const ce_cache* h, F&& f) {
   if (h->vec) f(RowTag<f32x4>{}); else f(RowTag<float>{});
 }
+
+static InvMap inv_map(const ce_cache* h) { return InvMap{h->cfg.inverted_cached_idx, h->id_slot, h->row_id}; }
 
 static PhaseProf* live_prof(const ce_cache* h) {
   return (h->prof && (const void*)h->prof == h->pend.prof) ? h->prof : nullptr;
@@ -533,7 +538,7 @@
                        (VT*)c.cache_weight, h->rowlen, h->g_log2, (const Ctl*)nullptr, 0ll);
   });
   hipLaunchKernelGGL(k_admit_maps, dim3(grid_for(n, 256)), dim3(256), 0, s, rows, (const int32_t*)nullptr,
-                     (const long long*)nullptr, (long long)n, c.cached_idx_map, c.inverted_cached_idx,
+                     (const long long*)nullptr, (long long)n, c.cached_idx_map, inv_map(h),
                      c.freq_cnter, freq_vals, h->slot_epoch, kEpochNever, (Ctl*)nullptr,
                      (ce_call_stats_t*)nullptr, 0ll, (const unsigned long long*)nullptr, 0ll);
   hipLaunchKernelGGL(k_preload_end, dim3(1), dim3(1), 0, s, (long long)n, h->ctl, h->ring_dev + (h->seq % kRing),
@@ -655,7 +660,7 @@
   if (k > 0) {
     int32_t* evicted_rows_dev = h->free_list;
     hipLaunchKernelGGL(k_evict_maps, dim3(grid_for(k, 256)), dim3(256), 0, s, h->victims, c.cached_idx_map,
-                       c.inverted_cached_idx, evicted_rows_dev, h->ctl);
+                       inv_map(h), evicted_rows_dev, h->ctl);
     CE_HIP_CHECK(hipMemcpyAsync(h->list_host, evicted_rows_dev, (size_t)k * 4, hipMemcpyDeviceToHost, s));
     const int64_t chunk = staged_chunk(h, k);
     for (int64_t off = 0; off < k; off += chunk) {
@@ -733,7 +738,7 @@
                                                      : EvTable{nullptr, nullptr, 0u};
     for_rows(h, [&](auto r) {
       using VT = typename decltype(r)::VT;
-      hipLaunchKernelGGL((k_evict_stage<VT>), sg, dim3(256), 0, s, h->victims, c.cached_idx_map, c.inverted_cached_idx,
+      hipLaunchKernelGGL((k_evict_stage<VT>), sg, dim3(256), 0, s, h->victims, c.cached_idx_map, inv_map(h),
                          (const VT*)c.cache_weight, (VT*)stage_cur, stage_idx_cur, scap, h->rowlen, h->g_log2, h->ctl, mail,
                          x.sel_out_job, sgrid, (const unsigned long long*)h->keys, C, (const int32_t*)h->blk_free, free_list,
                          evt, L.list_cap > L.stage_rows ? (VT*)c.host_weight_dev : (VT*)nullptr);
@@ -797,10 +802,14 @@
       const int U = n >= 65536 ? 2 : 1;
       const int threads = (int)std::min<int64_t>(1024, std::max<int64_t>(64, cdiv(cdiv(n, U), 64) * 64));
       const dim3 tg((unsigned)cdiv(n, (int64_t)threads * U)), tb(threads);
-#define CE_TOUCH(U_)                                                                                                \
-  hipLaunchKernelGGL((k_touch<U_>), tg, tb, 0, s, ids, n, c.idx_map, c.inverted_cached_idx, N, h->bitmap, h->fine_cnt, \
+      const bool map = h->id_slot != nullptr;
+      const int32_t* const slot_of = map ? h->id_slot : c.inverted_cached_idx;
+      h->pend.enc = map;
+#define CE_TOUCH(U_, MAP_)                                                                                          \
+  hipLaunchKernelGGL((k_touch<U_, MAP_>), tg, tb, 0, s, ids, n, c.idx_map, slot_of, N, h->bitmap, h->fine_cnt,       \
                      h->coarse_cnt, h->slot_epoch, seq_arg, fw, h->victims, (unsigned)L.list_cap, slots_out, allow_pad)
-      if (U == 2) CE_TOUCH(2); else CE_TOUCH(1);
+      if (map) { if (U == 2) CE_TOUCH(2, true); else CE_TOUCH(1, true); }
+      else { if (U == 2) CE_TOUCH(2, false); else CE_TOUCH(1, false); }
 #undef CE_TOUCH
     }
     const int rgrid = (int)std::min<int64_t>(kNumCU, std::max<int64_t>(1, cdiv(std::max(n, C), 4096)));
@@ -935,7 +944,7 @@
     phase_mark(h);
     StageArgs a;
     a.cached_idx_map = c.cached_idx_map;
-    a.inverted = c.inverted_cached_idx;
+    a.inv = inv_map(h);
     a.freq = c.freq_cnter;
     a.slot_epoch = h->slot_epoch;
     a.C = C;
@@ -977,7 +986,7 @@
     if (rc0) return rc0;
     hipLaunchKernelGGL(k_admit_maps, dim3(grid_for(L.list_cap, 256)), dim3(256), 0, s, h->miss_list_b[parity],
                        h->free_list_b[parity], (const long long*)&h->ctl->n_miss, 0ll, c.cached_idx_map,
-                       c.inverted_cached_idx, c.freq_cnter, (const int64_t*)nullptr, h->slot_epoch, 0, h->ctl,
+                       inv_map(h), c.freq_cnter, (const int64_t*)nullptr, h->slot_epoch, 0, h->ctl,
                        h->ring_dev, x.seq_arg, (const unsigned long long*)nullptr, 0ll, &h->chain->n_unpack[parity]);
     CE_HIP_CHECK(hipEventRecord(w->ev_miss[parity], s));
     sel_done = w->ev_miss[parity];
@@ -1028,6 +1037,7 @@
                "only the zero-copy transport can be captured in a hipGraph (the others hand rows to host threads)");
     CE_REQUIRE(!h->prof, CE_ERR_UNSUPPORTED, "switch the phase timers off before capturing a cache op");
     CE_REQUIRE(!split, CE_ERR_UNSUPPORTED, "a cache op in two halves cannot be captured in a hipGraph");
+    if (h->cfg.idx_map && !h->id_slot) h->captured_plain = true;
   }
   int rc = capturing ? CE_OK : before_call(h);
   if (rc) return rc;
@@ -1106,8 +1116,8 @@
   const KeysTail* const tail = x.has_tail ? &x.tail : nullptr;
   int rc = CE_OK;
   if (n > 0 && lfu) {
-    hipLaunchKernelGGL(k_slots_lfu, dim3(std::min(grid_for(n, 8192), kMaxBlocks)), dim3(1024), 0, s, slots_out, n,
-                       c.inverted_cached_idx, c.freq_cnter, (const Ctl*)h->ctl);
+    hipLaunchKernelGGL(x.enc ? k_slots_lfu<true> : k_slots_lfu<false>, dim3(std::min(grid_for(n, 8192), kMaxBlocks)),
+                       dim3(1024), 0, s, slots_out, n, c.inverted_cached_idx, c.freq_cnter, (const Ctl*)h->ctl);
     if (tail) {
       rc = tail->src_keys
                ? ce_bag_presort_window_src(slots_out, tail->nnz_per_batch, tail->n_batches, C, tail->lay.offsets,
@@ -1118,11 +1128,11 @@
     }
   } else if (n > 0 && tail) {
     rc = presort_window_from_rows(slots_out, tail->nnz_per_batch, tail->n_batches, C, c.inverted_cached_idx,
-                                  &h->ctl->status, tail->src_keys, tail->lay, tail->keys_out, s);
+                                  &h->ctl->status, tail->src_keys, tail->lay, tail->keys_out, s, x.enc);
     if (rc) return rc;
   } else if (n > 0) {
-    hipLaunchKernelGGL(k_slots, dim3(grid_for(n, 256 * 4)), dim3(256), 0, s, slots_out, n, c.inverted_cached_idx,
-                       (const Ctl*)h->ctl);
+    hipLaunchKernelGGL(x.enc ? k_slots<true> : k_slots<false>, dim3(grid_for(n, 256 * 4)), dim3(256), 0, s, slots_out, n,
+                       c.inverted_cached_idx, (const Ctl*)h->ctl);
   }
   phase_mark(h);
   return CE_OK;
@@ -1185,7 +1195,7 @@
   rc = x.worker ? admit_parked(h) : c.transport == CE_TRANSPORT_ZEROCOPY ? admit_zero_copy(h) : admit_staged(h);
   if (rc) return rc;
   hipLaunchKernelGGL(k_admit_maps, dim3(grid_for(h->L.list_cap, 256)), dim3(256), 0, s, h->miss_list, h->free_list,
-                     (const long long*)&h->ctl->n_miss, 0ll, c.cached_idx_map, c.inverted_cached_idx,
+                     (const long long*)&h->ctl->n_miss, 0ll, c.cached_idx_map, inv_map(h),
                      c.freq_cnter, (const int64_t*)nullptr, h->slot_epoch, 0, h->ctl, h->ring_dev,
                      x.seq_arg, x.worker ? (const unsigned long long*)(h->wb->sig_dev + 1) : nullptr, x.in_job);
   phase_mark(h);
@@ -1339,10 +1349,58 @@
   CE_REQUIRE(ids && slots_out && n > 0, CE_ERR_INVALID, "null ids/slots");
   const ce_cache_config_t& c = h->cfg;
   hipLaunchKernelGGL(k_lookup, dim3(grid_for(n, 256)), dim3(256), 0, (hipStream_t)stream, ids, n, c.idx_map,
-                     c.inverted_cached_idx, c.num_embeddings, slots_out);
+                     c.inverted_cached_idx, (const int32_t*)h->id_slot, c.num_embeddings, slots_out);
   CE_LAUNCH_CHECK();
   return CE_OK;
 }
+
+__global__ __launch_bounds__(256) void k_build_id_slot(const int32_t* __restrict__ idx_map,
+                                                       const int32_t* __restrict__ inverted, int64_t N,
+                                                       int32_t* __restrict__ id_slot, int32_t* __restrict__ row_id) {
+  const int64_t stride = (int64_t)gridDim.x * blockDim.x;
+  for (int64_t id = (int64_t)blockIdx.x * blockDim.x + threadIdx.x; id < N; id += stride) {
+    const int32_t row = idx_map[id];
+    if ((uint32_t)row >= (uint64_t)N) continue;
+    id_slot[id] = inverted[row];
+    row_id[row] = (int32_t)id;
+  }
+}
+
+extern "C" int ce_cache_set_id_slot_map(ce_cache_t* h, int32_t* id_slot, int32_t* row_id, ce_stream_t stream) {
+  CE_REQUIRE(h, CE_ERR_INVALID, "null handle");
+  CE_REQUIRE(!h->pend.active, CE_ERR_INVALID, "a cache op begun with ce_cache_prepare_ids_begin has not been finished");
+  CE_REQUIRE((id_slot == nullptr) == (row_id == nullptr), CE_ERR_INVALID, "id_slot and row_id come together (or both NULL)");
+  if (!id_slot) {
+    if (h->id_slot) {
+      const int rc = sync_and_drain(h);
+      if (rc) return rc;
+    }
+    h->id_slot = h->row_id = nullptr;
+    return CE_OK;
+  }
+  CE_REQUIRE(h->cfg.idx_map, CE_ERR_INVALID, "the handle has no idx_map: inverted_cached_idx is indexed by id already");
+  CE_REQUIRE(!h->captured_plain, CE_ERR_UNSUPPORTED,
+             "a cache op was captured into a hipGraph without the map: its replays would not maintain it");
+  hipStream_t s = (hipStream_t)stream;
+  hipStreamCaptureStatus cap_st = hipStreamCaptureStatusNone;
+  if (s != nullptr) CE_HIP_CHECK(hipStreamIsCapturing(s, &cap_st));
+  CE_REQUIRE(cap_st != hipStreamCaptureStatusActive, CE_ERR_UNSUPPORTED, "not capturable");
+  CE_HIP_CHECK(hipStreamWaitEvent(s, h->ev, 0));
+  const int rc = join_rows(h, s);
+  if (rc) return rc;
+  const int64_t N = h->cfg.num_embeddings;
+  hipLaunchKernelGGL(k_fill_i32, dim3(grid_for(N, 256 * 4)), dim3(256), 0, s, id_slot, N, -1);
+  hipLaunchKernelGGL(k_fill_i32, dim3(grid_for(N, 256 * 4)), dim3(256), 0, s, row_id, N, -1);
+  hipLaunchKernelGGL(k_build_id_slot, dim3(grid_for(N, 256 * 4)), dim3(256), 0, s, (const int32_t*)h->cfg.idx_map,
+                     (const int32_t*)h->cfg.inverted_cached_idx, N, id_slot, row_id);
+  CE_LAUNCH_CHECK();
+  CE_HIP_CHECK(hipEventRecord(h->ev, s));
+  h->id_slot = id_slot;
+  h->row_id = row_id;
+  return CE_OK;
+}
+
+extern "C" int32_t ce_cache_has_id_slot_map(ce_cache_t* h) { return (h && h->id_slot) ? 1 : 0; }
 
 extern "C" int ce_cache_flush(ce_cache_t* h, ce_stream_t stream) {
   CE_REQUIRE(h, CE_ERR_INVALID, "null handle");
@@ -1370,7 +1428,7 @@
                        (const VT*)c.cache_weight, (VT*)c.host_weight_dev, h->rowlen, h->g_log2);
   });
   hipLaunchKernelGGL(k_flush_maps, dim3(grid_for(C, 256)), dim3(256), 0, s, c.cached_idx_map, C,
-                     c.inverted_cached_idx, c.freq_cnter, h->slot_epoch, h->ctl);
+                     inv_map(h), c.freq_cnter, h->slot_epoch, h->ctl);
   hipLaunchKernelGGL(k_flush_end, dim3(1), dim3(1), 0, s, C, h->ctl, h->ring_dev + (h->seq % kRing),
                      (long long)h->seq);
   CE_LAUNCH_CHECK();
diff --git a/cachedembedding_amd/csrc/ce_cache_fused.h b/cachedembedding_amd/csrc/ce_cache_fused.h
--- a/cachedembedding_amd/csrc/ce_cache_fused.h
+++ b/cachedembedding_amd/csrc/ce_cache_fused.h
@@ -65,7 +65,7 @@
 }
 
 
-template <int U>
+template <int U, bool MAP>
 __global__ __launch_bounds__(1024) void k_touch(const int64_t* __restrict__ ids, int64_t n,
                                                const int32_t* __restrict__ idx_map,
                                                const int32_t* __restrict__ inverted, int64_t N, uint32_t* bitmap,
@@ -85,12 +85,16 @@
     const int64_t i = i0 + u * 64 + lane;
     valid[u] = i < n;
     row[u] = 0;
+    inv[u] = 0;
     if (valid[u]) {
       const int64_t id = ids[i];
       if ((unsigned long long)id >= (unsigned long long)N) {
         if (!(allow_pad && id == -1)) bad = true;
         valid[u] = false;
         rows_out[i] = -1;
+      } else if (MAP) {
+        row[u] = (int32_t)id;
+        inv[u] = inverted[id];
       } else {
         row[u] = idx_map ? idx_map[id] : (int32_t)id;
       }
@@ -98,8 +102,10 @@
   }
 #pragma unroll
   for (int u = 0; u < U; ++u) {
-    inv[u] = 0;
-    if (valid[u]) {
+    if (!valid[u]) continue;
+    if (MAP) {
+      if (inv[u] < 0) row[u] = idx_map[row[u]];
+    } else {
       rows_out[i0 + u * 64 + lane] = row[u];
       inv[u] = inverted[row[u]];
     }
@@ -109,6 +115,7 @@
   for (int u = 0; u < U; ++u) {
     first[u] = false;
     if (!valid[u]) continue;
+    if (MAP) rows_out[i0 + u * 64 + lane] = inv[u] >= 0 ? (int64_t)inv[u] : -2 - (int64_t)row[u];
     if (inv[u] >= 0) {
       slot_epoch[inv[u]] = epoch;
     } else {
@@ -287,7 +294,7 @@
 
 struct StageArgs {
   int32_t* cached_idx_map;
-  int32_t* inverted;
+  InvMap inv;
   int64_t* freq;
   int32_t* slot_epoch;
   int64_t C;
@@ -412,9 +419,9 @@
       const long long i = i0 + t;
       const bool staged = i < a.scap;
       if (gl == 0) {
-        a.inverted[old[t]] = -1;
+        inv_set(a.inv, old[t], -1);
         a.cached_idx_map[slot[t]] = in_row[t];
-        a.inverted[in_row[t]] = slot[t];
+        inv_set(a.inv, in_row[t], slot[t]);
         a.slot_epoch[slot[t]] = epoch;
         if (a.freq) a.freq[slot[t]] = 0;
         if (staged) {
diff --git a/cachedembedding_amd/csrc/ce_cache_rows.h b/cachedembedding_amd/csrc/ce_cache_rows.h
--- a/cachedembedding_amd/csrc/ce_cache_rows.h
+++ b/cachedembedding_amd/csrc/ce_cache_rows.h
@@ -9,9 +9,22 @@
 
 constexpr int kSwapRows = 16;
 
+struct InvMap {
+  int32_t* inverted;
+  int32_t* id_slot;
+  const int32_t* row_id;
+};
+__device__ __forceinline__ void inv_set(const InvMap& m, int64_t row, int32_t slot) {
+  m.inverted[row] = slot;
+  if (m.id_slot) {
+    const int32_t id = m.row_id[row];
+    if (id >= 0) m.id_slot[id] = slot;
+  }
+}
+
 template <typename VT>
 __global__ __launch_bounds__(1024) void k_evict(const int32_t* __restrict__ victims, int32_t* cached_idx_map,
-                                               int32_t* inverted, const VT* __restrict__ cache, VT* host,
+                                               InvMap inv, const VT* __restrict__ cache, VT* host,
                                                long long first, int rowlen, int g_log2, const Ctl* ctl) {
   const long long k = (ctl->status == CE_OK) ? ctl->k_evict : 0;
   if (k <= first) return;
@@ -38,7 +51,7 @@
         if (dst[t] < 0) continue;
         if (gl < rowlen) host[dst[t] * rowlen + gl] = v[t];
         if (gl == 0) {
-          inverted[dst[t]] = -1;
+          inv_set(inv, dst[t], -1);
           cached_idx_map[victims[i + t]] = -1;
         }
       }
@@ -49,7 +62,7 @@
         copy_row(cache + (int64_t)slot * rowlen, host + (int64_t)row * rowlen, rowlen, gl, G);
         __builtin_amdgcn_wave_barrier();
         if (gl == 0) {
-          inverted[row] = -1;
+          inv_set(inv, row, -1);
           cached_idx_map[slot] = -1;
         }
       }
@@ -138,7 +151,7 @@
 
 template <typename VT>
 __global__ __launch_bounds__(256) void k_evict_stage(const int32_t* __restrict__ victims,
-                                                     int32_t* cached_idx_map, int32_t* inverted,
+                                                     int32_t* cached_idx_map, InvMap inv,
                                                      const VT* __restrict__ cache, VT* stage, int32_t* stage_rows_idx,
                                                      long long cap, int rowlen, int g_log2, const Ctl* ctl,
                                                      WbMail* mail, long long job, int stage_grid,
@@ -163,7 +176,7 @@
       copy_row(cache + (int64_t)slot * rowlen, host_overflow + (int64_t)row * rowlen, rowlen, gl0, G0);
       __builtin_amdgcn_wave_barrier();
       if (gl0 == 0) {
-        inverted[row] = -1;
+        inv_set(inv, row, -1);
         cached_idx_map[slot] = -1;
       }
     }
@@ -188,7 +201,7 @@
         if (gl == 0) {
           const int32_t row = cached_idx_map[slot[t]];
           stage_rows_idx[i + t] = row;
-          inverted[row] = -1;
+          inv_set(inv, row, -1);
           cached_idx_map[slot[t]] = -1;
           if (evt.keys) evt_insert(evt, (uint32_t)job, row, (int32_t)(i + t));
         }
@@ -203,7 +216,7 @@
         if (gl == 0) {
           const int32_t row = cached_idx_map[slot];
           stage_rows_idx[i + t] = row;
-          inverted[row] = -1;
+          inv_set(inv, row, -1);
           cached_idx_map[slot] = -1;
           if (evt.keys) evt_insert(evt, (uint32_t)job, row, (int32_t)(i + t));
         }
@@ -246,14 +259,14 @@
 }
 
 __global__ __launch_bounds__(256) void k_evict_maps(const int32_t* __restrict__ victims, int32_t* cached_idx_map,
-                                                    int32_t* inverted, int32_t* evicted_rows, const Ctl* ctl) {
+                                                    InvMap inv, int32_t* evicted_rows, const Ctl* ctl) {
   const long long k = (ctl->status == CE_OK) ? ctl->k_evict : 0;
   const int64_t stride = (int64_t)gridDim.x * blockDim.x;
   for (int64_t i = (int64_t)blockIdx.x * blockDim.x + threadIdx.x; i < k; i += stride) {
     const int32_t slot = victims[i];
     const int32_t row = cached_idx_map[slot];
     if (evicted_rows) evicted_rows[i] = row;
-    inverted[row] = -1;
+    inv_set(inv, row, -1);
     cached_idx_map[slot] = -1;
   }
 }
@@ -483,7 +496,7 @@
 
 __global__ __launch_bounds__(256) void k_admit_maps(const int32_t* __restrict__ rows,
                                                     const int32_t* __restrict__ slots, const long long* n_ptr,
-                                                    long long n_imm, int32_t* cached_idx_map, int32_t* inverted,
+                                                    long long n_imm, int32_t* cached_idx_map, InvMap inv,
                                                     int64_t* freq, const int64_t* freq_vals, int32_t* slot_epoch,
                                                     int32_t epoch_imm, Ctl* ctl, ce_call_stats_t* ring,
                                                     long long seq_arg, const unsigned long long* fail_word,
@@ -511,7 +524,7 @@
     const int32_t row = rows ? rows[i] : (int32_t)i;
     const int32_t slot = slots ? slots[i] : (int32_t)i;
     cached_idx_map[slot] = row;
-    inverted[row] = slot;
+    inv_set(inv, row, slot);
     if (freq) freq[slot] = freq_vals ? freq_vals[i] : 0;
     slot_epoch[slot] = epoch;
   }
@@ -519,16 +532,19 @@
 
 __global__ __launch_bounds__(256) void k_lookup(const int64_t* __restrict__ ids, int64_t n,
                                                 const int32_t* __restrict__ idx_map,
-                                                const int32_t* __restrict__ inverted, int64_t N, int64_t* slots_out) {
+                                                const int32_t* __restrict__ inverted,
+                                                const int32_t* __restrict__ id_slot, int64_t N, int64_t* slots_out) {
   const int64_t stride = (int64_t)gridDim.x * blockDim.x;
   for (int64_t i = (int64_t)blockIdx.x * blockDim.x + threadIdx.x; i < n; i += stride) {
     const int64_t id = ids[i];
     int64_t slot = -1;
-    if ((unsigned long long)id < (unsigned long long)N) slot = inverted[idx_map ? idx_map[id] : (int32_t)id];
+    if ((unsigned long long)id < (unsigned long long)N)
+      slot = id_slot ? id_slot[id] : inverted[idx_map ? idx_map[id] : (int32_t)id];
     slots_out[i] = slot;
   }
 }
 
+template <bool ENC>
 __global__ __launch_bounds__(256) void k_slots(int64_t* slots, int64_t n, const int32_t* __restrict__ inverted,
                                                const Ctl* ctl) {
   const bool failed = ctl->status != CE_OK;
@@ -544,13 +560,14 @@
 #pragma unroll
     for (int u = 0; u < U; ++u) {
       const int64_t i = i0 + (int64_t)u * blockDim.x;
-      if (i < n) slots[i] = (failed || row[u] < 0) ? -1 : (int64_t)inverted[row[u]];
+      if (i < n) slots[i] = failed ? -1 : (int64_t)front_slot<ENC>(row[u], inverted);
     }
   }
 }
 
 constexpr int kSlotsHashBits = 13;
 constexpr int kSlotsHash = 1 << kSlotsHashBits;
+template <bool ENC>
 __global__ __launch_bounds__(1024) void k_slots_lfu(int64_t* slots, int64_t n, const int32_t* __restrict__ inverted,
                                                     int64_t* freq, const Ctl* ctl) {
   __shared__ int hkey[kSlotsHash];
@@ -571,7 +588,7 @@
       row[u] = (i < hi && !failed) ? slots[i] : -1;
     }
 #pragma unroll
-    for (int u = 0; u < U; ++u) slot[u] = row[u] >= 0 ? inverted[row[u]] : -1;
+    for (int u = 0; u < U; ++u) slot[u] = front_slot<ENC>(row[u], inverted);
 #pragma unroll
     for (int u = 0; u < U; ++u) {
       const int64_t i = i0 + (int64_t)u * blockDim.x;
@@ -609,14 +626,14 @@
   }
 }
 
-__global__ __launch_bounds__(256) void k_flush_maps(int32_t* cached_idx_map, int64_t C, int32_t* inverted,
+__global__ __launch_bounds__(256) void k_flush_maps(int32_t* cached_idx_map, int64_t C, InvMap inv,
                                                     int64_t* freq, int32_t* slot_epoch, Ctl* ctl) {
   const int64_t stride = (int64_t)gridDim.x * blockDim.x;
   int n = 0;
   for (int64_t s = (int64_t)blockIdx.x * blockDim.x + threadIdx.x; s < C; s += stride) {
     const int32_t row = cached_idx_map[s];
     if (row >= 0) {
-      inverted[row] = -1;
+      inv_set(inv, row, -1);
       cached_idx_map[s] = -1;
       ++n;
     }
diff --git a/cachedembedding_amd/csrc/ce_common.h b/cachedembedding_amd/csrc/ce_common.h
--- a/cachedembedding_amd/csrc/ce_common.h
+++ b/cachedembedding_amd/csrc/ce_common.h
@@ -84,9 +84,15 @@
   int64_t hook_features;
 };
 
+template <bool ENC>
+__device__ __forceinline__ int32_t front_slot(int64_t v, const int32_t* __restrict__ inverted) {
+  if (ENC) return v >= 0 ? (int32_t)v : (v <= -2 ? inverted[-2 - v] : -1);
+  return v >= 0 ? inverted[v] : -1;
+}
+
 int presort_window_from_rows(int64_t* slots_io, int64_t nnz_per_batch, int64_t n_batches, int64_t num_rows,
                              const int32_t* inverted, const int* status, int32_t src_keys, const BagLayout& lay,
-                             uint64_t* keys_out, hipStream_t stream);
+                             uint64_t* keys_out, hipStream_t stream, bool encoded = false);
 
 void bind_thread_near_gpu();
 bool near_gpu_cpus(cpu_set_t* out);
diff --git a/include/ce_api.h b/include/ce_api.h
--- a/include/ce_api.h
+++ b/include/ce_api.h
@@ -345,6 +345,9 @@
 int ce_cache_lookup_slots(ce_cache_t* h, const int64_t* ids, int64_t n, int64_t* slots_out,
                           ce_stream_t stream);
 
+int ce_cache_set_id_slot_map(ce_cache_t* h, int32_t* id_slot, int32_t* row_id, ce_stream_t stream);
+int32_t ce_cache_has_id_slot_map(ce_cache_t* h);
+
 int ce_cache_flush(ce_cache_t* h, ce_stream_t stream);
 
 int ce_cache_set_protect_depth(ce_cache_t* h, int32_t depth);
```

Measured after the change: 3.144 billion. -1.8%, worse.
